# victorkich/ManyTor

Hardware: AMD Instinct MI355X
Metric: env-steps/sec (whole node), 1M parallel 4-DoF arms, random actions (higher is better)
Workload: dtype f32

## Files before the change

manytor_amd/csrc/engine.hip:

```cpp
#include <hip/hip_runtime.h>

#include <algorithm>
#include <cmath>
#include <cstdio>
#include <cstdlib>
#include <cstring>
#include <mutex>
#include <new>
#include <iterator>
#include <string>
#include <utility>
#include <vector>

#include "engine_internal.h"
#include "kernels.h"

using namespace mt;

namespace {
thread_local std::string g_last_error;
}

namespace mt {
int fail(mt_handle h, int code, const std::string& msg) {
  if (h)
    h->err = msg;
  else
    g_last_error = msg;
  return code;
}

int join_chains(mt_handle h) {
  if (!h->forked) return MT_OK;
  h->forked = false;
  for (int c = 1; c < mt_engine::kMaxChains; ++c) {
    if (!h->chain_streams[c] || !h->ev_join[c]) continue;
    MT_HIP(h, hipEventRecord(h->ev_join[c], h->chain_streams[c]));
    MT_HIP(h, hipStreamWaitEvent(h->stream, h->ev_join[c], 0));
  }
  return MT_OK;
}
}

namespace {

DhConst make_dh(const float* table, int dof) {
  DhConst t{};
  for (int j = 0; j < MT_MAX_DOF; ++j) {
    t.ca[j] = 1.f;
  }
  for (int j = 0; j < dof; ++j) {
    const double a = table[4 * j + 0], alpha = table[4 * j + 1], d = table[4 * j + 2], off = table[4 * j + 3];
    t.a[j] = (float)a;
    t.d[j] = (float)d;
    double sa = std::sin(alpha), ca = std::cos(alpha);
    if (std::fabs(sa) < 1e-7) sa = 0.0;
    if (std::fabs(ca) < 1e-7) ca = 0.0;
    t.sa[j] = (float)sa;
    t.ca[j] = (float)ca;
    t.off_deg[j] = (float)(off * 180.0 / M_PI);
  }
  t.fo = dof >= 2 ? dof - 2 : 0;
  t.fe = dof - 1;
  return t;
}

size_t align_up(size_t v, size_t a) { return (v + a - 1) / a * a; }

int ensure_staging(mt_handle h, size_t bytes) {
  if (h->staging_bytes >= bytes) return MT_OK;
  if (h->staging) {
    MT_HIP(h, hipStreamSynchronize(h->stream));
    MT_HIP(h, hipFree(h->staging));
    h->staging = nullptr;
    h->staging_bytes = 0;
  }
  if (hipMalloc(&h->staging, bytes) != hipSuccess) return fail(h, MT_ERR_ALLOC, "hipMalloc(staging) failed");
  h->staging_bytes = bytes;
  return MT_OK;
}

template <class Tbl>
bool table_matches(const DhConst& t, int dof) {
  if (dof != Tbl::D) return false;
  for (int j = 0; j < dof; ++j)
    if (t.a[j] != Tbl::a(j) || t.d[j] != Tbl::d(j) || t.sa[j] != Tbl::sa(j) || t.ca[j] != Tbl::ca(j) ||
        t.off_deg[j] != Tbl::off(j))
      return false;
  return true;
}

int match_static(const DhConst& t, int dof) {
  if (table_matches<Ref4Table>(t, dof)) return 1;
  if (table_matches<Dh7Table>(t, dof)) return 2;
  return 0;
}

struct BlockCap {
  int64_t from, below;
  int blocks;
};
struct DispatchPolicy {
  int64_t step_split4_max = 49152, step_split2_max = 65536;
  int64_t prefetch_other_max = 131072;
  int64_t fused_split4_max = 32768, fused_split2_max = 131072;
  int64_t reset_split_max = 65536;
  int64_t graph_max = 131072;
  int64_t chains_min = 163840, chains_max = 3145728;
  int64_t chain_split4_max = 16384, chain_split2_max = 49152, chain_prefetch_other_max = 131072;
  int64_t flat_from = 393216;
  BlockCap block_caps[3] = {{147456, 229376, 3}, {229376, 458752, 4}, {458752, 589824, 5}};
  int64_t multi_step_max = 262144;
  int multi_step_k = 5;
  bool fold_reset_into_chains = false;
  int max_recurrence_rotations = 12;
  int64_t ld_pad_above = 16384;
  int ld_pad_floats = 256;
};
static const DispatchPolicy kPolicy{};

static int step_blocks_per_cu(const mt_engine* h, int64_t n_launch) {
  if (h->blocks_per_cu_override >= 0) return h->blocks_per_cu_override;
  if (n_launch >= h->n) return 0;
  for (const BlockCap& c : kPolicy.block_caps)
    if (n_launch >= c.from && n_launch < c.below) return c.blocks;
  return 0;
}
static size_t lds_pad_for_blocks(int blocks_per_cu, size_t static_lds) {
  if (blocks_per_cu <= 0) return 0;
  const size_t per_block = (size_t)163840 / (size_t)blocks_per_cu - 1024;
  return per_block > static_lds ? std::min<size_t>(per_block, 65536) - static_lds : 0;
}

int64_t chain_span(const mt_engine* h, int chains) {
  const int64_t per = (h->n + chains - 1) / chains;
  return (per + 255) / 256 * 256;
}

static bool env_int(const char* name, long long* v) {
  const char* e = std::getenv(name);
  if (!e || !*e) return false;
  *v = std::atoll(e);
  return true;
}

static void choose_dispatch(mt_handle h) {
  const mt_config* cfg = &h->cfg;
  const DispatchPolicy& P = kPolicy;
  const int64_t n = cfg->n_envs;
  long long v = 0;
  h->overrides.clear();
  auto seen = [&](const char* name) { h->overrides += (h->overrides.empty() ? "" : ",") + std::string(name) + "=" + std::to_string(v); };

  h->trig = (cfg->flags & MT_FLAG_HW_TRIG) ? 2 : ((cfg->flags & MT_FLAG_DIRECT_TRIG) ? 1 : 0);
  if (cfg->flags & MT_FLAG_ABLATE_LOOP) h->trig = (cfg->flags & MT_FLAG_ABLATE_OBS) ? 4 : 3;
  else if (cfg->flags & MT_FLAG_ABLATE_OBS) h->trig = 5;
  const bool long_route = h->trig == 0 && (cfg->substeps - 1) / 2 > P.max_recurrence_rotations;
  if (long_route) h->trig = 1;
  h->lds_table = (cfg->flags & MT_FLAG_DH_IN_LDS) != 0 && !long_route;
  h->custom_frames = !(h->args.dh.fo == h->D - 2 && h->args.dh.fe == h->D - 1);
  h->static_kind = ((cfg->flags & (MT_FLAG_NO_SPECIALIZE | MT_FLAG_DH_IN_LDS)) || h->custom_frames) ? 0 : match_static(h->args.dh, h->D);

  int forced_lanes = 0, forced_prefetch = -1;
  if (env_int("MT_SPLIT", &v)) {
    forced_lanes = (v == 2 || v == 4) ? (int)v : 1;
    seen("MT_SPLIT");
  }
  if (env_int("MT_PREFETCH", &v)) {
    forced_prefetch = v != 0;
    seen("MT_PREFETCH");
  }
  h->reset_split = n <= P.reset_split_max;
  if (env_int("MT_RESET_SPLIT", &v)) {
    h->reset_split = v != 0;
    seen("MT_RESET_SPLIT");
  }
  h->graph_mode = -1;
  h->graph_max = P.graph_max;
  if (env_int("MT_GRAPH", &v)) {
    h->graph_mode = v != 0 ? 1 : 0;
    seen("MT_GRAPH");
  }
  h->flat_from = P.flat_from;
  if (env_int("MT_FLAT_FROM", &v)) {
    h->flat_from = std::max<long long>(0, v);
    seen("MT_FLAT_FROM");
  }
  h->blocks_per_cu_override = -1;
  if (env_int("MT_BLOCKS_PER_CU", &v)) {
    const int c = (int)std::max<long long>(0, std::min<long long>(8, v));
    h->blocks_per_cu_override = (c == 1 || c == 2) ? 3 : c;
    seen("MT_BLOCKS_PER_CU");
  }
  h->trig_steps = h->static_kind != 0;
  if (env_int("MT_TRIG_TABLE", &v)) {
    h->trig_steps = v != 0 && h->static_kind != 0;
    seen("MT_TRIG_TABLE");
  }

  h->chains = (n >= P.chains_min && n <= P.chains_max) ? 2 : 1;
  h->chains_forced = false;
  if (env_int("MT_CHAINS", &v)) {
    h->chains = (int)std::max<long long>(1, std::min<long long>(mt_engine::kMaxChains, v));
    h->chains_forced = true;
    seen("MT_CHAINS");
  }
  if (n < 2 * 256) h->chains = 1;
  h->lazy_chains = true;
  if (env_int("MT_LAZY_CHAINS", &v)) {
    h->lazy_chains = v != 0;
    seen("MT_LAZY_CHAINS");
  }

  h->multi_k = (n <= P.multi_step_max) ? P.multi_step_k : 1;
  if (env_int("MT_ROLLOUT_K", &v)) {
    h->multi_k = (int)std::max<long long>(1, std::min<long long>(64, v));
    seen("MT_ROLLOUT_K");
  }
  h->defer_reset = true;
  if (env_int("MT_DEFER_RESET", &v)) {
    h->defer_reset = v != 0;
    seen("MT_DEFER_RESET");
  }
  h->defer_reset_chained = P.fold_reset_into_chains;
  if (env_int("MT_DEFER_RESET_CHAINS", &v)) {
    h->defer_reset_chained = v != 0;
    seen("MT_DEFER_RESET_CHAINS");
  }
  h->gather_throttle = true;
  if (env_int("MT_GATHER_THROTTLE", &v)) {
    h->gather_throttle = v != 0;
    seen("MT_GATHER_THROTTLE");
  }
  h->snap_in_rollout = true;
  if (env_int("MT_ROLLOUT_SNAP", &v)) {
    h->snap_in_rollout = v != 0;
    seen("MT_ROLLOUT_SNAP");
  }
  h->rollout_early = true;
  if (env_int("MT_ROLLOUT_EARLY", &v)) {
    h->rollout_early = v != 0;
    seen("MT_ROLLOUT_EARLY");
  }

  h->tape_prefetch = false;
  if (env_int("MT_TAPE_PREFETCH", &v)) {
    h->tape_prefetch = v != 0;
    seen("MT_TAPE_PREFETCH");
  }
  h->tape_nt_loads = false;
  if (env_int("MT_TAPE_NT", &v)) {
    h->tape_nt_loads = v != 0;
    seen("MT_TAPE_NT");
  }

  h->ground_compact = true;
  if (env_int("MT_GROUND_COMPACT", &v)) {
    h->ground_compact = v != 0;
    seen("MT_GROUND_COMPACT");
  }

  if (h->custom_frames) h->lds_table = false;
  auto schedule_for = [&](int64_t envs, int64_t split4_max, int64_t split2_max, int64_t prefetch_other_max) {
    mt_engine::Schedule s;
    s.step_lanes = envs <= split4_max ? 4 : (envs <= split2_max ? 2 : 1);
    s.prefetch = h->static_kind == 1 || envs <= prefetch_other_max;
    s.rollout_lanes = envs <= P.fused_split4_max ? 4 : (envs <= P.fused_split2_max ? 2 : 1);
    if (forced_lanes) s.step_lanes = s.rollout_lanes = forced_lanes;
    if (forced_prefetch >= 0) s.prefetch = forced_prefetch != 0;
    if (h->custom_frames) s = mt_engine::Schedule{};
    return s;
  };
  h->sched[mt_engine::kBatch] = schedule_for(n, P.step_split4_max, P.step_split2_max, P.prefetch_other_max);
  h->sched[mt_engine::kChain] =
      h->chains > 1 ? schedule_for(chain_span(h, h->chains), P.chain_split4_max, P.chain_split2_max, P.chain_prefetch_other_max)
                    : h->sched[mt_engine::kBatch];
}

#define MT_DISPATCH_D(D_, FN, ...)   \
  switch (D_) {                      \
    case 2: FN<2>(__VA_ARGS__); break; \
    case 3: FN<3>(__VA_ARGS__); break; \
    case 4: FN<4>(__VA_ARGS__); break; \
    case 5: FN<5>(__VA_ARGS__); break; \
    case 6: FN<6>(__VA_ARGS__); break; \
    case 7: FN<7>(__VA_ARGS__); break; \
    case 8: FN<8>(__VA_ARGS__); break; \
    default: break;                  \
  }

struct StepVariant {
  int trig = 0;
  bool lds = false;
  int lanes = 1;
  int pf = 0;
  bool tt = false;
  bool flat = false;
  bool fresh = false;
  bool codes = false;
  bool gc = false;
};
constexpr unsigned variant_key(const StepVariant& v) {
  return (unsigned)v.trig | (unsigned)v.lds << 3 | (unsigned)v.lanes << 4 | (unsigned)(v.pf != 0) << 7 | (unsigned)v.tt << 8 |
         (unsigned)v.flat << 9 | (unsigned)v.fresh << 10 | (unsigned)v.codes << 11 | (unsigned)v.gc << 12;
}

#pragma clang diagnostic push
#pragma clang diagnostic ignored "-Wc++20-designator"
constexpr StepVariant kRuntimeVariants[] = {
    {.trig = 0}, {.trig = 1}, {.trig = 2}, {.trig = 3}, {.trig = 4}, {.trig = 5},
    {.lds = true},
    {.lanes = 2}, {.lanes = 4},
    {.pf = kPrefetch}, {.pf = kPrefetch, .flat = true},
    {.gc = true}, {.pf = kPrefetch, .gc = true}, {.pf = kPrefetch, .flat = true, .gc = true},
};
constexpr StepVariant kFramesVariants[] = {{.trig = 0}, {.trig = 1}};
constexpr StepVariant kStaticVariants[] = {
    {.trig = 0}, {.trig = 1}, {.trig = 2}, {.trig = 3}, {.trig = 4}, {.trig = 5},
    {.lanes = 2}, {.lanes = 4},
    {.lanes = 2, .tt = true}, {.lanes = 4, .tt = true},
    {.pf = kPrefetch}, {.pf = kPrefetch, .flat = true},
    {.pf = 0, .tt = true}, {.pf = kPrefetch, .tt = true}, {.pf = kPrefetch, .tt = true, .flat = true},
    {.pf = kPrefetch, .tt = true, .codes = true}, {.pf = kPrefetch, .tt = true, .flat = true, .codes = true},
    {.pf = 0, .tt = true, .fresh = true}, {.pf = kPrefetch, .tt = true, .fresh = true},
    {.pf = kPrefetch, .tt = true, .flat = true, .fresh = true},
    {.gc = true}, {.pf = kPrefetch, .gc = true}, {.pf = kPrefetch, .flat = true, .gc = true},
    {.pf = 0, .tt = true, .gc = true}, {.pf = kPrefetch, .tt = true, .gc = true}, {.pf = kPrefetch, .tt = true, .flat = true, .gc = true},
    {.pf = kPrefetch, .tt = true, .codes = true, .gc = true}, {.pf = kPrefetch, .tt = true, .flat = true, .codes = true, .gc = true},
};
#pragma clang diagnostic pop

enum class TableKind { kRuntime = 0, kRef4 = 1, kDh7 = 2, kFrames = 3 };
struct StepPlan {
  TableKind table = TableKind::kRuntime;
  int D = 0;
  bool sample = false;
  StepVariant v;
  int blocks_per_cu = 0;
  size_t lds_bytes = 0;
  dim3 grid;
  bool exists = true;
};

static bool ground_compacts(const mt_engine* h, bool whole_rows) {
  return h->ground_compact && whole_rows && h->trig == 0 && !h->lds_table && !h->custom_frames &&
         !(h->cfg.flags & MT_FLAG_DEBUG_ZMIN) && h->D <= 5;
}
template <int D>
static void ground_queue_bytes_d(size_t* out) { *out = sizeof(GroundQueue<RtTable<D>>); }
static size_t ground_queue_bytes(const mt_engine* h) {
  if (h->static_kind == 1) return sizeof(GroundQueue<Ref4Table>);
  if (h->static_kind == 2) return sizeof(GroundQueue<Dh7Table>);
  size_t bytes = 0;
  MT_DISPATCH_D(h->D, ground_queue_bytes_d, &bytes);
  return bytes;
}

StepPlan plan_step(const mt_engine* h, mt_engine::Scope scope, int64_t n, bool sample, bool codes, bool fresh = false) {
  const mt_engine::Schedule& s = h->sched[scope == mt_engine::kChain ? mt_engine::kChain : mt_engine::kBatch];
  const bool whole_rows = scope != mt_engine::kOneEnv;
  StepPlan p;
  p.table = h->custom_frames ? TableKind::kFrames : (TableKind)h->static_kind;
  p.D = h->D;
  p.sample = sample;
  p.grid = grid_for(n);
  StepVariant& v = p.v;
  if (fresh) {
    const size_t stage = (size_t)2 * h->K * kBlock * sizeof(float), fixed = kTrigEntries * sizeof(SinCos) + 512;
    p.exists = h->trig == 0 && h->trig_steps && s.step_lanes == 1 && !h->lds_table && !h->trace &&
               stage + fixed <= 65536;
    if (!p.exists) return p;
    p.sample = true;
    v.tt = v.fresh = true;
    v.pf = s.prefetch ? kPrefetch : 0;
    v.flat = v.pf && n >= h->flat_from;
    p.blocks_per_cu = v.pf ? step_blocks_per_cu(h, n) : 0;
    p.lds_bytes = std::max(stage, lds_pad_for_blocks(p.blocks_per_cu, fixed));
    return p;
  }
  if (p.table == TableKind::kFrames) {
    v.trig = h->trig == 1 ? 1 : 0;
    return p;
  }
  if (h->lds_table) {
    v.lds = true;
    return p;
  }
  if (h->trig != 0) {
    v.trig = h->trig;
    return p;
  }
  v.tt = sample && h->trig_steps && whole_rows;
  if (s.step_lanes > 1) {
    v.lanes = s.step_lanes;
    const int64_t per_block = kBlock / v.lanes;
    p.grid = dim3((unsigned)((n + per_block - 1) / per_block));
    return p;
  }
  v.pf = s.prefetch ? kPrefetch : 0;
  v.flat = v.pf && n >= h->flat_from;
  v.codes = v.pf && v.tt && codes;
  v.gc = ground_compacts(h, whole_rows);
  if (v.pf && v.tt) {
    p.blocks_per_cu = step_blocks_per_cu(h, n);
    p.lds_bytes = lds_pad_for_blocks(p.blocks_per_cu, kTrigEntries * sizeof(SinCos) + (v.gc ? ground_queue_bytes(h) : 0));
  }
  return p;
}

template <class Tbl, bool SAMPLE, const auto& ROWS, size_t I>
void launch_variant(const StepPlan& p, hipStream_t stream, const StepArgs& args) {
  constexpr StepVariant V = ROWS[I];
  if constexpr (V.lanes > 1)
    hipLaunchKernelGGL((step_split_kernel<Tbl, SAMPLE, V.lanes, V.tt>), p.grid, dim3(kBlock), p.lds_bytes, stream, args);
  else
    hipLaunchKernelGGL((step_kernel<Tbl, SAMPLE, V.trig, V.lds, V.pf, V.tt, V.flat, V.fresh, V.codes, V.gc>), p.grid, dim3(kBlock),
                       p.lds_bytes, stream, args);
}
template <class Tbl, const auto& ROWS, size_t I>
bool launch_row(const StepPlan& p, hipStream_t stream, const StepArgs& args) {
  if (variant_key(p.v) != variant_key(ROWS[I])) return false;
  if constexpr (ROWS[I].gc && Tbl::D >= 6)
    return false;
  else if (p.sample)
    launch_variant<Tbl, true, ROWS, I>(p, stream, args);
  else if constexpr (!ROWS[I].tt)
    launch_variant<Tbl, false, ROWS, I>(p, stream, args);
  else
    return false;
  return true;
}
template <class Tbl, const auto& ROWS, size_t... I>
bool launch_rows(const StepPlan& p, hipStream_t stream, const StepArgs& args, std::index_sequence<I...>) {
  return (launch_row<Tbl, ROWS, I>(p, stream, args) || ...);
}
template <class Tbl, const auto& ROWS>
bool launch_table(const StepPlan& p, hipStream_t stream, const StepArgs& args) {
  return launch_rows<Tbl, ROWS>(p, stream, args, std::make_index_sequence<std::size(ROWS)>{});
}
template <int D>
void launch_plan_d(const StepPlan& p, hipStream_t stream, const StepArgs& args, bool* launched) {
  *launched = p.table == TableKind::kFrames ? launch_table<RtTableF<D>, kFramesVariants>(p, stream, args)
                                            : launch_table<RtTable<D>, kRuntimeVariants>(p, stream, args);
}

void launch_plan(const StepPlan& p, hipStream_t stream, const StepArgs& args) {
  bool launched = false;
  if (p.v.gc && (int64_t)p.grid.x * kBlock > args.ld) {
    std::fprintf(stderr, "manytor: a ground-compacting step launch of %u blocks over rows of %lld\n", p.grid.x, (long long)args.ld);
    std::abort();
  }
  if (p.table == TableKind::kRef4)
    launched = launch_table<Ref4Table, kStaticVariants>(p, stream, args);
  else if (p.table == TableKind::kDh7)
    launched = launch_table<Dh7Table, kStaticVariants>(p, stream, args);
  else
    MT_DISPATCH_D(p.D, launch_plan_d, p, stream, args, &launched);
  if (!launched) {
    std::fprintf(stderr, "manytor: no step kernel for table %d, D %d, sample %d, variant key 0x%x\n", (int)p.table, p.D,
                 (int)p.sample, variant_key(p.v));
    std::abort();
  }
}

template <int D>
void launch_trace_d(mt_handle h, const StepArgs& args, float* trace, bool sample) {
  if (sample)
    hipLaunchKernelGGL((trace_kernel<D, true>), grid_for(args.n), dim3(kBlock), 0, h->stream, args, trace);
  else
    hipLaunchKernelGGL((trace_kernel<D, false>), grid_for(args.n), dim3(kBlock), 0, h->stream, args, trace);
}

void launch_step(mt_handle h, mt_engine::Scope scope, const StepArgs& args, float* trace, bool sample) {
  if (trace) MT_DISPATCH_D(h->D, launch_trace_d, h, args, trace, sample);
  const StepPlan p = plan_step(h, scope, args.n, sample, h->codes_valid);
  launch_plan(p, h->stream, args);
  h->codes_valid = p.v.codes;
}

void launch_step(mt_handle h, bool sample) { launch_step(h, mt_engine::kBatch, h->args, h->trace, sample); }

bool launch_step_fresh(mt_handle h, mt_engine::Scope scope, const StepArgs& args) {
  const StepPlan p = plan_step(h, scope, args.n, true, false, true);
  if (!p.exists) return false;
  launch_plan(p, h->stream, args);
  h->codes_valid = p.v.codes;
  return true;
}

StepArgs args_for_range(mt_handle h, const StepArgs& base, int64_t off, int64_t cnt);
int check_launch(mt_handle h, const char* what);
int ensure_chains(mt_handle h, int chains) {
  if (!h->ev_fork) MT_HIP(h, hipEventCreateWithFlags(&h->ev_fork, event_flags(false)));
  for (int c = 1; c < chains; ++c) {
    if (!h->chain_streams[c]) MT_HIP(h, hipStreamCreateWithFlags(&h->chain_streams[c], hipStreamNonBlocking));
    if (!h->ev_join[c]) MT_HIP(h, hipEventCreateWithFlags(&h->ev_join[c], event_flags(false)));
  }
  return MT_OK;
}

void launch_chain(mt_handle h, const StepArgs& a0, uint32_t major0, int T, int chains, int c, bool sample = true) {
  const int64_t span = chain_span(h, chains), off = (int64_t)c * span;
  if (off >= h->n) return;
  StepArgs as = args_for_range(h, a0, off, std::min(span, h->n - off));
  for (int s = 0; s < T; ++s) {
    as.major = major0 + (uint32_t)s;
    launch_step(h, mt_engine::kChain, as, nullptr, sample);
  }
}

bool launch_chain_fresh(mt_handle h, const StepArgs& a0, uint32_t major, int chains, int c) {
  const int64_t span = chain_span(h, chains), off = (int64_t)c * span;
  if (off >= h->n) return true;
  StepArgs as = args_for_range(h, a0, off, std::min(span, h->n - off));
  as.major = major;
  return launch_step_fresh(h, mt_engine::kChain, as);
}

hipStream_t chain_stream(mt_handle h, int c) { return c == 0 ? h->stream : h->chain_streams[c]; }

int fork_chains(mt_handle h, int chains) {
  if (h->forked) return MT_OK;
  int rc = ensure_chains(h, chains);
  if (rc) return rc;
  const int64_t span = chain_span(h, chains);
  MT_HIP(h, hipEventRecord(h->ev_fork, h->stream));
  for (int c = 1; c < chains; ++c)
    if ((int64_t)c * span < h->n) MT_HIP(h, hipStreamWaitEvent(h->chain_streams[c], h->ev_fork, 0));
  h->forked = true;
  return MT_OK;
}

int settle_chains(mt_handle h) { return (h->lazy_chains && h->stream == h->own_stream) ? MT_OK : join_chains(h); }

void shift_rows(StepArgs& a, int64_t off) {
  a.actions += off;
  a.goals += off;
  a.points += off;
  a.codes += off;
  a.alive += off;
  a.total_reward += off;
  a.obs += off;
  a.reward += off;
  a.done += off;
  a.ee += off;
  a.episodes += off;
  a.last_return += off;
  if (a.ring) a.ring += off;
  if (a.zmin) a.zmin += off;
  a.env_base += off;
}

StepArgs args_for_env(mt_handle h, int64_t env) {
  StepArgs a = h->args;
  shift_rows(a, env);
  a.done_bits = h->spare_bits;
  a.snap = nullptr;
  a.n = 1;
  return a;
}

StepArgs args_for_range(mt_handle h, const StepArgs& base, int64_t off, int64_t cnt) {
  StepArgs a = base;
  shift_rows(a, off);
  a.done_bits += off / 64;
  if (a.snap) a.snap += off;
  a.n = cnt;
  return a;
}

template <int D, bool RANDOM, bool ONLY_DONE>
void launch_reset_k(mt_handle h, const StepArgs& args) {
  const size_t lds = RANDOM ? (size_t)2 * args.K * kBlock * sizeof(float) : 0;
  if (lds > 65536)
    (void)hipFuncSetAttribute(reinterpret_cast<const void*>(&reset_kernel<D, RANDOM, ONLY_DONE>),
                              hipFuncAttributeMaxDynamicSharedMemorySize, (int)lds);
  hipLaunchKernelGGL((reset_kernel<D, RANDOM, ONLY_DONE>), grid_for(args.n), dim3(kBlock), lds, h->stream, args,
                     h->cfg.radius);
}
template <int D, bool ONLY_DONE>
void launch_reset_split(mt_handle h, const StepArgs& args) {
  constexpr int L = 4;
  const int64_t per_block = kBlock / L;
  const size_t lds = (size_t)2 * args.K * per_block * sizeof(float);
  hipLaunchKernelGGL((reset_split_kernel<D, ONLY_DONE, L>), dim3((unsigned)((args.n + per_block - 1) / per_block)),
                     dim3(kBlock), lds, h->stream, args, h->cfg.radius);
}
template <int D>
void launch_reset_d(mt_handle h, const StepArgs& args, int mode) {
  if (mode == 0) h->codes_valid = false;
  if (mode != 0 && h->reset_split && args.n == h->n)
    return mode == 1 ? launch_reset_split<D, false>(h, args) : launch_reset_split<D, true>(h, args);
  if (mode == 0)
    launch_reset_k<D, false, false>(h, args);
  else if (mode == 1)
    launch_reset_k<D, true, false>(h, args);
  else
    launch_reset_k<D, true, true>(h, args);
}

template <int D>
void launch_observe_d(mt_handle h) {
  hipLaunchKernelGGL((observe_kernel<D>), grid_for(h->n), dim3(kBlock), 0, h->stream, h->args);
}
template <int D>
void launch_check_done_d(mt_handle h) {
  hipLaunchKernelGGL((check_done_kernel<D>), grid_for(h->n), dim3(kBlock), 0, h->stream, h->args);
}
template <int D>
void launch_joints_d(mt_handle h, float* out) {
  hipLaunchKernelGGL((joints_kernel<D>), grid_for(h->n), dim3(kBlock), 0, h->stream, h->args, out);
}

template <class Tbl, int L, int RPF>
void launch_rollout_split_t(mt_handle h, const StepArgs& a, const RolloutArgs& r) {
  const int64_t per_block = kBlock / L;
  const size_t lds = (size_t)3 * h->K * per_block * sizeof(float) + (ActionTrigTable<Tbl>::value ? kTrigEntries * sizeof(SinCos) : 0);
  if (lds > 65536)
    (void)hipFuncSetAttribute(reinterpret_cast<const void*>(&rollout_split_kernel<Tbl, L, RPF>),
                              hipFuncAttributeMaxDynamicSharedMemorySize, (int)lds);
  hipLaunchKernelGGL((rollout_split_kernel<Tbl, L, RPF>), dim3((unsigned)((a.n + per_block - 1) / per_block)), dim3(kBlock), lds,
                     h->stream, a, r);
}

template <class Tbl, int RPF>
void launch_rollout_t(mt_handle h, const StepArgs& a, int lanes, const RolloutArgs& r) {
  if (lanes == 4) return launch_rollout_split_t<Tbl, 4, RPF>(h, a, r);
  if (lanes == 2) return launch_rollout_split_t<Tbl, 2, RPF>(h, a, r);
  const size_t lds = (size_t)3 * h->K * kBlock * sizeof(float) + (ActionTrigTable<Tbl>::value ? kTrigEntries * sizeof(SinCos) : 0);
  if (lds > 65536)
    (void)hipFuncSetAttribute(reinterpret_cast<const void*>(&rollout_kernel<Tbl, RPF>),
                              hipFuncAttributeMaxDynamicSharedMemorySize, (int)lds);
  hipLaunchKernelGGL((rollout_kernel<Tbl, RPF>), grid_for(a.n), dim3(kBlock), lds, h->stream, a, r);
}

template <int D>
void launch_rollout_d(mt_handle h, const StepArgs& a, int lanes, const RolloutArgs& r) {
  launch_rollout_t<RtTable<D>, 0>(h, a, lanes, r);
}
void launch_rollout(mt_handle h, const StepArgs& a, int lanes, const RolloutArgs& r, bool early = false) {
  h->codes_valid = false;
  if (h->static_kind == 1) return early ? launch_rollout_t<Ref4Table, kPrefetch>(h, a, lanes, r) : launch_rollout_t<Ref4Table, 0>(h, a, lanes, r);
  if (h->static_kind == 2) return early ? launch_rollout_t<Dh7Table, kPrefetch>(h, a, lanes, r) : launch_rollout_t<Dh7Table, 0>(h, a, lanes, r);
  MT_DISPATCH_D(h->D, launch_rollout_d, h, a, lanes, r);
}

template <class Tbl, bool PREFETCH>
void launch_tape_t(mt_handle h, const StepArgs& a, const TapeArgs& r) {
  const size_t lds = (size_t)3 * h->K * kBlock * sizeof(float);
  if (lds > 65536)
    (void)hipFuncSetAttribute(reinterpret_cast<const void*>(&rollout_tape_kernel<Tbl, PREFETCH>),
                              hipFuncAttributeMaxDynamicSharedMemorySize, (int)lds);
  hipLaunchKernelGGL((rollout_tape_kernel<Tbl, PREFETCH>), grid_for(a.n), dim3(kBlock), lds, h->stream, a, r);
}
template <int D>
void launch_tape_d(mt_handle h, const StepArgs& a, const TapeArgs& r) {
  launch_tape_t<RtTable<D>, false>(h, a, r);
}
bool tape_prefetches(const mt_engine* h) { return h->tape_prefetch && h->static_kind != 0; }
void launch_tape(mt_handle h, const StepArgs& a, const TapeArgs& r) {
  const bool pf = tape_prefetches(h);
  if (h->static_kind == 1) return pf ? launch_tape_t<Ref4Table, true>(h, a, r) : launch_tape_t<Ref4Table, false>(h, a, r);
  if (h->static_kind == 2) return pf ? launch_tape_t<Dh7Table, true>(h, a, r) : launch_tape_t<Dh7Table, false>(h, a, r);
  MT_DISPATCH_D(h->D, launch_tape_d, h, a, r);
}

template <class Tbl>
struct TableTag {
  using type = Tbl;
};
template <class F>
void with_table(const mt_engine* h, F&& f) {
  if (h->static_kind == 1) return f(TableTag<Ref4Table>{});
  if (h->static_kind == 2) return f(TableTag<Dh7Table>{});
  switch (h->D) {
    case 2: return f(TableTag<RtTable<2>>{});
    case 3: return f(TableTag<RtTable<3>>{});
    case 4: return f(TableTag<RtTable<4>>{});
    case 5: return f(TableTag<RtTable<5>>{});
    case 6: return f(TableTag<RtTable<6>>{});
    case 7: return f(TableTag<RtTable<7>>{});
    case 8: return f(TableTag<RtTable<8>>{});
    default: return;
  }
}

template <class Tbl>
void launch_tape_select_t(mt_handle h, const StepArgs& a, const TapeArgs& r) {
  const size_t lds = (size_t)3 * h->K * kBlock * sizeof(float);
  if (lds > 65536)
    (void)hipFuncSetAttribute(reinterpret_cast<const void*>(&rollout_tape_kernel<Tbl, false, true>),
                              hipFuncAttributeMaxDynamicSharedMemorySize, (int)lds);
  hipLaunchKernelGGL((rollout_tape_kernel<Tbl, false, true>), grid_for(a.n), dim3(kBlock), lds, h->stream, a, r);
}
void launch_tape_select(mt_handle h, const StepArgs& a, const TapeArgs& r) {
  with_table(h, [&](auto tag) { launch_tape_select_t<typename decltype(tag)::type>(h, a, r); });
}

template <class Tbl, int W>
void launch_policy_t(mt_handle h, const StepArgs& a, const PolicyArgs& r) {
  const size_t lds = (size_t)3 * h->K * kBlock * sizeof(float);
  if (lds > 65536)
    (void)hipFuncSetAttribute(reinterpret_cast<const void*>(&rollout_policy_kernel<Tbl, W>),
                              hipFuncAttributeMaxDynamicSharedMemorySize, (int)lds);
  hipLaunchKernelGGL((rollout_policy_kernel<Tbl, W>), grid_for(a.n), dim3(kBlock), lds, h->stream, a, r);
}
void launch_policy(mt_handle h, const StepArgs& a, const PolicyArgs& r, int width) {
  with_table(h, [&](auto tag) {
    using Tbl = typename decltype(tag)::type;
    if (width <= 32) return launch_policy_t<Tbl, 32>(h, a, r);
    launch_policy_t<Tbl, 64>(h, a, r);
  });
}


template <class Tbl>
void launch_shoot_t(mt_handle h, const StepArgs& a, const ShootArgs& r) {
  const size_t lds = ((size_t)3 * h->K + 2 * kShootWaves) * kShootEnvs * sizeof(float);
  hipLaunchKernelGGL((shoot_kernel<Tbl>), dim3((unsigned)((a.n + kShootEnvs - 1) / kShootEnvs)), dim3(kBlock), lds, h->stream, a, r);
}
void launch_shoot(mt_handle h, const StepArgs& a, const ShootArgs& r) {
  with_table(h, [&](auto tag) { launch_shoot_t<typename decltype(tag)::type>(h, a, r); });
}

template <class Tbl>
void launch_cem_t(mt_handle h, const StepArgs& a, const CemArgs& r) {
  const size_t lds = ((size_t)3 * h->K + (size_t)r.C + 2 * kShootWaves + 1) * kShootEnvs * sizeof(float);
  hipLaunchKernelGGL((cem_kernel<Tbl>), dim3((unsigned)((a.n + kShootEnvs - 1) / kShootEnvs)), dim3(kBlock), lds, h->stream, a, r);
}
void launch_cem(mt_handle h, const StepArgs& a, const CemArgs& r) {
  with_table(h, [&](auto tag) { launch_cem_t<typename decltype(tag)::type>(h, a, r); });
}

template <class Tbl>
void launch_mppi_t(mt_handle h, const StepArgs& a, const MppiArgs& r) {
  const size_t lds = (((size_t)3 * h->K + (size_t)r.C) * kShootEnvs + kMppiTable) * sizeof(float);
  hipLaunchKernelGGL((mppi_kernel<Tbl>), dim3((unsigned)((a.n + kShootEnvs - 1) / kShootEnvs)), dim3(kBlock), lds, h->stream, a, r);
}
void launch_mppi(mt_handle h, const StepArgs& a, const MppiArgs& r) {
  with_table(h, [&](auto tag) { launch_mppi_t<typename decltype(tag)::type>(h, a, r); });
}

template <int D>
void launch_sample_plans_d(mt_handle h, const CemArgs& r, float* plans, int64_t ld, int64_t cand_stride) {
  hipLaunchKernelGGL((sample_plans_kernel<D>), dim3(grid_for(h->n).x, (unsigned)r.T, (unsigned)r.C), dim3(kBlock), 0, h->stream, r, plans,
                     ld, cand_stride, h->args.n, h->args.env_base);
}

bool fusable(mt_handle h) { return h->trig == 0 && !h->lds_table && !h->trace && !h->custom_frames; }
const char* unfusable_reason(const mt_engine* h) {
  return h->custom_frames                        ? "custom obs_frame / ee_frame"
         : h->trace                              ? "MT_FLAG_TRACE"
         : h->lds_table                          ? "MT_FLAG_DH_IN_LDS"
         : h->trig == 2                          ? "MT_FLAG_HW_TRIG"
         : (h->cfg.flags & MT_FLAG_DIRECT_TRIG) ? "MT_FLAG_DIRECT_TRIG"
         : h->trig == 1                          ? "substeps beyond the recurrence's reach (per-pose trigonometry)"
                                                 : "a profiling flag (MT_FLAG_ABLATE_*)";
}
int fail_unfusable(mt_handle h, const char* who) {
  return fail(h, MT_ERR_UNSUPPORTED, std::string(who) + ": not available on a handle with " + unfusable_reason(h));
}

bool rollout_is_multi_step(mt_handle h) { return h->multi_k > 1 && fusable(h); }
bool chained_rollout_absorbs_reset(mt_handle h) {
  const bool graph = h->graph_mode > 0 || (h->graph_mode < 0 && h->n <= h->graph_max);
  return h->defer_reset_chained && !rollout_is_multi_step(h) && h->chains > 1 && h->lazy_chains && !h->trace && !graph && fusable(h);
}


int check_launch(mt_handle h, const char* what) {
  hipError_t e = hipGetLastError();
  if (e != hipSuccess) return fail(h, MT_ERR_HIP, std::string(what) + " launch: " + hipGetErrorString(e));
  return MT_OK;
}

struct FieldInfo {
  void* ptr;
  int rows;
  int dtype;
  size_t esize;
};

int field_info(mt_handle h, int field, FieldInfo* fi) {
  const StepArgs& a = h->args;
  switch (field) {
    case MT_F_ACTIONS: *fi = {a.actions, h->D, MT_F32, 4}; return MT_OK;
    case MT_F_GOALS: *fi = {a.goals, h->D, MT_F32, 4}; return MT_OK;
    case MT_F_POINTS: *fi = {a.points, 3 * h->K, MT_F32, 4}; return MT_OK;
    case MT_F_ALIVE: *fi = {a.alive, 1, MT_U32, 4}; return MT_OK;
    case MT_F_OBS: *fi = {a.obs, 3 * h->K, MT_F32, 4}; return MT_OK;
    case MT_F_REWARD: *fi = {a.reward, 1, MT_I32, 4}; return MT_OK;
    case MT_F_DONE: *fi = {a.done, 1, MT_U8, 1}; return MT_OK;
    case MT_F_DONE_BITS: *fi = {a.done_bits, 1, MT_U64, 8}; return MT_OK;
    case MT_F_EE: *fi = {a.ee, 3, MT_F32, 4}; return MT_OK;
// ... 262 lines not shown
  };
#define MT_HIP_C(call)                                                                       \
  do {                                                                                       \
    hipError_t e__ = (call);                                                                 \
    if (e__ != hipSuccess) return bail(MT_ERR_HIP, std::string(#call) + ": " + hipGetErrorString(e__)); \
  } while (0)

  DeviceGuard guard(cfg->device);
  if (guard.error() != hipSuccess) return bail(MT_ERR_HIP, std::string("hipSetDevice: ") + hipGetErrorString(guard.error()));
  MT_HIP_C(hipStreamCreateWithFlags(&h->own_stream, hipStreamNonBlocking));
  h->stream = h->own_stream;
  MT_HIP_C(hipEventCreateWithFlags(&h->ev0, event_flags(true)));
  MT_HIP_C(hipEventCreateWithFlags(&h->ev1, event_flags(true)));

  const size_t ld = (size_t)h->ld, D = (size_t)h->D, K = (size_t)h->K;
  size_t off = 0;
  auto take = [&](size_t bytes) {
    size_t o = off;
    off = align_up(off + bytes, 1024);
    return o;
  };
  const size_t o_act = take(D * ld * 4), o_goal = take(D * ld * 4), o_pts = take(3 * K * ld * 4),
               o_obs = take(3 * K * ld * 4), o_alive = take(ld * 4), o_tot = take(ld * 4), o_rew = take(ld * 4),
               o_done = take(ld), o_bits = take(ld / 64 * 8), o_ee = take(3 * ld * 4), o_epi = take(ld * 4),
               o_last = take(ld * 4), o_ring = take((size_t)cfg->return_ring * ld * 4), o_misc = take(256),
               o_trace = take((cfg->flags & MT_FLAG_TRACE) ? (size_t)cfg->substeps * 3 * ld * 4 : 0),
               o_zmin = take((cfg->flags & MT_FLAG_DEBUG_ZMIN) ? ld * 4 : 0), o_trig = take(kTrigEntries * sizeof(SinCos)),
               o_codes = take(2 * K * ld * 4);
  h->arena_bytes = off;
  if (hipMalloc(&h->arena, h->arena_bytes) != hipSuccess) {
    (void)hipGetLastError();
    return bail(MT_ERR_ALLOC, "hipMalloc of the state arena failed (" + std::to_string(h->arena_bytes) + " bytes)");
  }
  MT_HIP_C(hipMemsetAsync(h->arena, 0, h->arena_bytes, h->stream));
  char* base = (char*)h->arena;
  StepArgs& a = h->args;
  a.actions = (float*)(base + o_act);
  a.goals = (float*)(base + o_goal);
  a.points = (float*)(base + o_pts);
  a.codes = (uint32_t*)(base + o_codes);
  a.obs = (float*)(base + o_obs);
  a.alive = (uint32_t*)(base + o_alive);
  a.total_reward = (float*)(base + o_tot);
  a.reward = (int32_t*)(base + o_rew);
  a.done = (uint8_t*)(base + o_done);
  a.done_bits = (unsigned long long*)(base + o_bits);
  a.ee = (float*)(base + o_ee);
  a.episodes = (uint32_t*)(base + o_epi);
  a.last_return = (float*)(base + o_last);
  a.ring = cfg->return_ring ? (float*)(base + o_ring) : nullptr;
  a.ring_slots = (uint32_t)cfg->return_ring;
  a.episode0 = 0;
  a.bad_actions = (uint32_t*)(base + o_misc);
  h->spare_bits = (unsigned long long*)(base + o_misc + 64);
  h->trace = (cfg->flags & MT_FLAG_TRACE) ? (float*)(base + o_trace) : nullptr;
  a.zmin = (cfg->flags & MT_FLAG_DEBUG_ZMIN) ? (float*)(base + o_zmin) : nullptr;
  a.snap = nullptr;
  a.trig_table = (const float*)(base + o_trig);
  hipLaunchKernelGGL(fill_trig_table_kernel, dim3(1), dim3(kBlock), 0, h->stream, (float*)(base + o_trig));
  MT_HIP_C(hipGetLastError());
  a.n = h->n;
  a.ld = h->ld;
  a.env_base = cfg->env_id_base;
  a.K = h->K;
  a.S = cfg->substeps;
  a.tol = cfg->pickup_tol;
  a.radius = cfg->radius;
  a.inv_sm1 = 1.0f / (float)(cfg->substeps - 1);
  a.flags = cfg->flags & ~kFlagWholeGoals;
  a.dh = make_dh(cfg->dh_table, h->D);
  a.dh.fo = (cfg->obs_frame + h->D) % h->D;
  a.dh.fe = (cfg->ee_frame + h->D) % h->D;
  choose_dispatch(h);
#undef MT_HIP_C
  *out = h;
  return MT_OK;
}

int mt_destroy(mt_handle h) {
  if (!h) return MT_OK;
  DeviceGuard guard(h->cfg.device);
  (void)hipStreamSynchronize(h->stream);
  mt_gather_release(h);
  mt_comm_release(h);
  for (auto& g : h->graphs)
    for (hipGraphExec_t x : g.exec)
      if (x) (void)hipGraphExecDestroy(x);
  for (int c = 1; c < mt_engine::kMaxChains; ++c) {
    if (h->chain_streams[c]) {
      (void)hipStreamSynchronize(h->chain_streams[c]);
      (void)hipStreamDestroy(h->chain_streams[c]);
    }
    if (h->ev_join[c]) (void)hipEventDestroy(h->ev_join[c]);
    if (h->ev1c[c]) (void)hipEventDestroy(h->ev1c[c]);
  }
  if (h->ev_fork) (void)hipEventDestroy(h->ev_fork);
  if (h->graph_step0) (void)hipFree(h->graph_step0);
  if (h->staging) (void)hipFree(h->staging);
  if (h->pinned) (void)hipHostFree(h->pinned);
  if (h->arena) (void)hipFree(h->arena);
  if (h->ev0) (void)hipEventDestroy(h->ev0);
  if (h->ev1) (void)hipEventDestroy(h->ev1);
  for (hipEvent_t e : h->lap_events) (void)hipEventDestroy(e);
  if (h->own_stream) (void)hipStreamDestroy(h->own_stream);
  delete h;
  return MT_OK;
}

static StepPlan batch_plan(const mt_engine* h) { return plan_step(h, mt_engine::kBatch, h->n, true, false); }
static StepPlan chain_plan(const mt_engine* h) { return plan_step(h, mt_engine::kChain, chain_span(h, h->chains), true, false); }
static std::string table_name(const mt_engine* h) {
  const char* tbl = h->static_kind == 1 ? "Ref4Table" : (h->static_kind == 2 ? "Dh7Table" : nullptr);
  return tbl ? tbl : (h->custom_frames ? "RtTableF<" : "RtTable<") + std::to_string(h->D) + ">";
}
static int multi_step_lanes(const mt_engine* h) {
  return h->sched[(h->chains > 1 && h->chains_forced) ? mt_engine::kChain : mt_engine::kBatch].rollout_lanes;
}

const char* mt_step_kernel_name(mt_handle h) {
  if (!h) return "";
  const std::string table = table_name(h);
  const StepVariant v = batch_plan(h).v;
  if (v.lanes > 1)
    h->kernel_name = "step_split_kernel<" + table + ", L=" + std::to_string(v.lanes) + (v.tt ? ", tt=1>" : ">");
  else
    h->kernel_name = "step_kernel<" + table + ", trig=" + std::to_string(h->trig) + ", lds=" + (v.lds ? "true" : "false") +
                     ", pf=" + std::to_string(v.pf) + (v.tt ? ", tt=1" : "") + (v.flat ? ", flat=1>" : ">");
  const bool multi_one_chain = h->multi_k > 1 && fusable(h) && !h->chains_forced;
  if (h->chains > 1 && !multi_one_chain) {
    const StepPlan c = chain_plan(h);
    h->kernel_name += " [mt_rollout: " + std::to_string(h->chains) + " chains of " + std::to_string(chain_span(h, h->chains)) +
                      " envs, " + (c.v.lanes > 1 ? "L=" + std::to_string(c.v.lanes)
                                                 : "pf=" + std::to_string(c.v.pf) + (c.v.flat ? ", flat=1" : "")) +
                      (c.blocks_per_cu > 0 ? ", " + std::to_string(c.blocks_per_cu) + " blocks/CU" : std::string()) + "]";
  }
  if (h->multi_k > 1 && fusable(h)) {
    const int sp = multi_step_lanes(h);
    h->kernel_name += " [mt_rollout: " + std::to_string(h->multi_k) + " steps per launch, " +
                      (sp > 1 ? "rollout_split_kernel L=" + std::to_string(sp) : std::string("rollout_kernel")) + "]";
  }
  return h->kernel_name.c_str();
}

const char* mt_describe_dispatch(mt_handle h) {
  if (!h) return "";
  const DispatchPolicy& P = kPolicy;
  auto num = [](long long v) { return std::to_string(v); };
  auto b = [](bool v) { return std::string(v ? "true" : "false"); };
  const int64_t span = chain_span(h, h->chains);
  const std::string table = table_name(h);
  const StepPlan sb = batch_plan(h), sc = chain_plan(h);
  const bool multi = h->multi_k > 1 && fusable(h);
  const bool graph = h->graph_mode > 0 || (h->graph_mode < 0 && h->n <= h->graph_max);
  std::string caps = "[";
  for (const BlockCap& c : P.block_caps) caps += std::string(caps.size() > 1 ? "," : "") + "[" + num(c.from) + "," + num(c.below) + "," + num(c.blocks) + "]";
  caps += "]";
  std::string& d = h->describe;
  d = "{\"n_envs\":" + num(h->n) + ",\"ld\":" + num(h->ld) + ",\"dof\":" + num(h->D) + ",\"targets\":" + num(h->K) +
      ",\"table\":\"" + table + "\",\"trig\":" + num(h->trig) + ",\"lds_table\":" + b(h->lds_table) + ",\"custom_frames\":" + b(h->custom_frames) +
      ",\"step\":{\"lanes_per_env\":" + num(sb.v.lanes) + ",\"prefetch\":" + b(sb.v.pf != 0) +
      ",\"trig_table\":" + b(sb.v.tt) + ",\"flat\":" + b(sb.v.flat) + "}" +
      ",\"chains\":{\"count\":" + num(h->chains) + ",\"span\":" + num(h->chains > 1 ? span : h->n) + ",\"lazy\":" + b(h->lazy_chains) +
      ",\"lanes_per_env\":" + num(sc.v.lanes) + ",\"prefetch\":" + b(sc.v.pf != 0) + ",\"flat\":" + b(sc.v.flat) +
      ",\"blocks_per_cu\":" + num(h->chains > 1 ? sc.blocks_per_cu : 0) + "}" +
      ",\"rollout\":{\"form\":\"" + (multi ? "multi_step" : (h->chains > 1 ? "chained_steps" : (graph ? "graph_replay" : "launch_per_step"))) +
      "\",\"steps_per_launch\":" + num(multi ? h->multi_k : 1) + ",\"graph\":" + b(!multi && graph) +
      ",\"lanes_per_env\":" + num(multi ? multi_step_lanes(h) : (h->chains > 1 ? sc : sb).v.lanes) +
      ",\"chains\":" + num(multi && !h->chains_forced ? 1 : h->chains) +
      ",\"absorbs_reset\":" + b(h->defer_reset && (multi || chained_rollout_absorbs_reset(h))) + ",\"writes_snapshot\":" + b(h->snap_in_rollout && (multi || (h->chains > 1 && !graph && !h->trace))) + "}" +
      ",\"fused\":{\"usable\":" + b(fusable(h)) + ",\"lanes_per_env\":" + num(h->sched[mt_engine::kBatch].rollout_lanes) + "}" +
      ",\"tape\":{\"usable\":" + b(fusable(h)) + ",\"lanes_per_env\":1,\"chains\":1,\"prefetch\":" + b(tape_prefetches(h)) +
      ",\"nt_loads\":" + b(h->tape_nt_loads) + "}" +
      ",\"shoot\":{\"usable\":" + b(fusable(h)) + ",\"envs_per_block\":" + num(kShootEnvs) + ",\"waves_per_block\":" + num(kShootWaves) + "}" +
      ",\"cem\":{\"usable\":" + b(fusable(h)) + ",\"envs_per_block\":" + num(kShootEnvs) + ",\"waves_per_block\":" + num(kShootWaves) +
      ",\"max_candidates\":64}" +
      ",\"mppi\":{\"usable\":" + b(fusable(h)) + ",\"envs_per_block\":" + num(kShootEnvs) + ",\"waves_per_block\":" + num(kShootWaves) +
      ",\"max_candidates\":64,\"max_steps\":" + num(kMppiMaxSteps) + "}" +
      ",\"policy_rollout\":{\"usable\":" + b(fusable(h)) + ",\"lanes_per_env\":1,\"hidden_extents\":[32,64]}" +
      ",\"reset\":{\"lanes_per_env\":" + num(h->reset_split ? 4 : 1) + "}" +
      ",\"ground_compact\":{\"enabled\":" + b(h->ground_compact) + ",\"step\":" + b(sb.v.gc) + ",\"chains\":" + b(sc.v.gc) + "}" +
      ",\"overrides\":\"" + h->overrides + "\"" +
      ",\"policy\":{\"step_split4_max\":" + num(P.step_split4_max) + ",\"step_split2_max\":" + num(P.step_split2_max) +
      ",\"prefetch_other_max\":" + num(P.prefetch_other_max) + ",\"fused_split4_max\":" + num(P.fused_split4_max) +
      ",\"fused_split2_max\":" + num(P.fused_split2_max) + ",\"reset_split_max\":" + num(P.reset_split_max) +
      ",\"graph_max\":" + num(P.graph_max) + ",\"chains_min\":" + num(P.chains_min) + ",\"chains_max\":" + num(P.chains_max) +
      ",\"chain_split4_max\":" + num(P.chain_split4_max) + ",\"chain_split2_max\":" + num(P.chain_split2_max) +
      ",\"chain_prefetch_other_max\":" + num(P.chain_prefetch_other_max) + ",\"flat_from\":" + num(P.flat_from) +
      ",\"block_caps\":" + caps + ",\"multi_step_max\":" + num(P.multi_step_max) + ",\"multi_step_k\":" + num(P.multi_step_k) +
      ",\"max_recurrence_rotations\":" + num(P.max_recurrence_rotations) + ",\"ld_pad_above\":" + num(P.ld_pad_above) +
      ",\"ld_pad_floats\":" + num(P.ld_pad_floats) + "}" +
      ",\"arena_bytes\":" + num((long long)h->arena_bytes) + "}";
  return d.c_str();
}

int mt_set_stream(mt_handle h, void* hip_stream) {
  MT_REQUIRE(nullptr, h != nullptr, "handle is NULL");
  MT_ENTER(h);
  MT_HIP(h, hipStreamSynchronize(h->stream));
  h->stream = (hipStream_t)hip_stream;
  return MT_OK;
}

int mt_use_own_stream(mt_handle h) {
  MT_REQUIRE(nullptr, h != nullptr, "handle is NULL");
  MT_ENTER(h);
  MT_HIP(h, hipStreamSynchronize(h->stream));
  h->stream = h->own_stream;
  return MT_OK;
}

int mt_sync(mt_handle h) {
  MT_REQUIRE(nullptr, h != nullptr, "handle is NULL");
  MT_ENTER(h);
  MT_HIP(h, hipStreamSynchronize(h->stream));
  if (h->gather_pending) {
    MT_HIP(h, hipStreamSynchronize(h->side_stream));
    MT_HIP(h, hipEventElapsedTime(&h->last_gather_ms, h->ev_g0, h->ev_g1));
    h->gather_pending = false;
    h->snap_free_known[0] = h->snap_free_known[1] = true;
  }
  return MT_OK;
}

int mt_reset(mt_handle h, const float* points, int layout, int is_device) {
  MT_REQUIRE(nullptr, h != nullptr, "handle is NULL");
  MT_REQUIRE(h, points != nullptr, "points is NULL (use mt_reset_random for device-drawn targets)");
  MT_REQUIRE(h, layout == MT_ENV_MAJOR || layout == MT_SOA, "bad layout");
  if (!is_device && layout == MT_ENV_MAJOR) {
    const int64_t bad = first_unusable(points, h->n * 3 * h->K, kMaxFiniteBits);
    if (bad >= 0) return fail(h, MT_ERR_INVALID_ARG, "mt_reset: points element " + std::to_string(bad) + " is NaN or infinite");
  }
  if (!is_device && layout == MT_SOA)
    for (int r = 0; r < 3 * h->K; ++r) {
      const int64_t bad = first_unusable(points + (int64_t)r * h->ld, h->n, kMaxFiniteBits);
      if (bad >= 0)
        return fail(h, MT_ERR_INVALID_ARG, "mt_reset: points row " + std::to_string(r) + " element " + std::to_string(bad) + " is NaN or infinite");
    }
  MT_ENTER(h);
  const int rows = 3 * h->K;
  if (layout == MT_SOA) {
    const size_t bytes = (size_t)rows * h->ld * 4;
    MT_HIP(h, hipMemcpyAsync(h->args.points, points, bytes, is_device ? hipMemcpyDeviceToDevice : hipMemcpyHostToDevice,
                             h->stream));
  } else {
    const size_t bytes = (size_t)rows * h->n * 4;
    const float* src = points;
    if (!is_device) {
      int rc = ensure_staging(h, bytes);
      if (rc) return rc;
      MT_HIP(h, hipMemcpyAsync(h->staging, points, bytes, hipMemcpyHostToDevice, h->stream));
      src = (const float*)h->staging;
    }
    hipLaunchKernelGGL((env_major_to_soa<float>), grid_for(h->n), dim3(kBlock), 0, h->stream, src, rows, h->n,
                       h->args.points, h->ld);
    int rc = check_launch(h, "env_major_to_soa");
    if (rc) return rc;
  }
  {
    int rcg = order_behind_inplace_gather(h, h->stream);
    if (rcg) return rcg;
  }
  h->args.major = 0;
  h->args.episode0 = 0;
  if (!h->goals_exposed) h->args.flags |= kFlagWholeGoals;
  MT_DISPATCH_D(h->D, launch_reset_d, h, h->args, 0);
  int rc = check_launch(h, "reset_kernel");
  if (rc) return rc;
  if (!is_device) MT_HIP(h, hipStreamSynchronize(h->stream));
  h->is_reset = true;
  return MT_OK;
}

static int launch_reset_random(mt_handle h, uint64_t seed, uint32_t episode, int mode) {
  const bool per_chain = mode == 1 && h->chains > 1 && h->lazy_chains && h->forked;
  if (!per_chain) {
    int rc = join_chains(h);
    if (rc) return rc;
  }
  h->args.seed_lo = (uint32_t)seed;
  h->args.seed_hi = (uint32_t)(seed >> 32);
  h->args.major = episode;
  if (mode == 1) {
    h->args.episode0 = episode;
    if (!h->goals_exposed) h->args.flags |= kFlagWholeGoals;
  }
  if (per_chain) {
    int rc = fork_chains(h, h->chains);
    if (rc) return rc;
    const int64_t span = chain_span(h, h->chains);
    hipStream_t root = h->stream;
    for (int c = 0; c < h->chains && rc == MT_OK; ++c) {
      const int64_t off = (int64_t)c * span;
      if (off >= h->n) continue;
      const StepArgs ar = args_for_range(h, h->args, off, std::min(span, h->n - off));
      h->stream = c == 0 ? root : h->chain_streams[c];
      rc = order_behind_inplace_gather(h, h->stream);
      if (rc == MT_OK) MT_DISPATCH_D(h->D, launch_reset_d, h, ar, 1);
    }
    h->stream = root;
    if (rc == MT_OK) rc = check_launch(h, "reset_kernel (per chain)");
    if (rc) return rc;
    h->codes_valid = !h->points_exposed;
    h->is_reset = true;
    return settle_chains(h);
  }
  int rc = order_behind_inplace_gather(h, h->stream);
  if (rc) return rc;
  MT_DISPATCH_D(h->D, launch_reset_d, h, h->args, mode);
  rc = check_launch(h, "reset_kernel");
  if (rc) return rc;
  if (mode == 1) h->codes_valid = !h->points_exposed;
  h->is_reset = true;
  return MT_OK;
}

}

namespace mt {
int flush_pending_reset(mt_handle h) {
  if (!h->reset_pending) return MT_OK;
  h->reset_pending = false;
  return launch_reset_random(h, h->pend_seed, h->pend_episode, 1);
}
}

extern "C" {

static int reset_random_impl(mt_handle h, uint64_t seed, uint32_t episode, int mode) {
  MT_REQUIRE(nullptr, h != nullptr, "handle is NULL");
  MT_ON_DEVICE(h, h->cfg.device);
  h->snap_valid = false;
  int rc = flush_pending_reset(h);
  if (rc) return rc;
  if (mode == 1 && h->defer_reset && h->stream == h->own_stream &&
      ((rollout_is_multi_step(h) && !h->forked) || chained_rollout_absorbs_reset(h))) {
    h->args.seed_lo = (uint32_t)seed;
    h->args.seed_hi = (uint32_t)(seed >> 32);
    h->args.major = episode;
    h->args.episode0 = episode;
    if (!h->goals_exposed) h->args.flags |= kFlagWholeGoals;
    h->reset_pending = true;
    h->pend_seed = seed;
    h->pend_episode = episode;
    h->is_reset = true;
    return MT_OK;
  }
  return launch_reset_random(h, seed, episode, mode);
}

int mt_reset_random(mt_handle h, uint64_t seed, uint32_t episode) { return reset_random_impl(h, seed, episode, 1); }

int mt_reset_done(mt_handle h, uint64_t seed) {
  MT_REQUIRE(nullptr, h != nullptr, "handle is NULL");
  if (!h->is_reset) return fail(h, MT_ERR_STATE, "mt_reset_done before the first reset");
  return reset_random_impl(h, seed, 0, 2);
}

int mt_set_actions(mt_handle h, const void* actions, int dtype, int layout, int is_device) {
  MT_REQUIRE(nullptr, h != nullptr, "handle is NULL");
  MT_REQUIRE(h, actions != nullptr, "actions is NULL");
  MT_REQUIRE(h, layout == MT_ENV_MAJOR || layout == MT_SOA, "bad layout");
  MT_REQUIRE(h, dtype == MT_F32 || dtype == MT_F64 || dtype == MT_I32 || dtype == MT_I64, "bad action dtype");
  const size_t es = (dtype == MT_F32 || dtype == MT_I32) ? 4 : 8;
  const int chains = is_device ? usable_chains(h, true) : 1;
  if (chains > 1) {
    MT_ON_DEVICE(h, h->cfg.device);
    const int D = h->D;
    const int64_t ld = h->ld;
    hipError_t copy_err = hipSuccess;
    int rc = per_chain(h, chains, "set_actions (per chain)", [&](int, int64_t off, int64_t cnt) {
      const dim3 g = grid_for(cnt), b(kBlock);
      float* dst = h->args.actions + off;
      if (layout == MT_SOA && dtype == MT_F32) {
        hipError_t e = hipMemcpy2DAsync(dst, (size_t)ld * 4, (const float*)actions + off, (size_t)ld * 4, (size_t)cnt * 4, (size_t)D,
                                        hipMemcpyDeviceToDevice, h->stream);
        if (e != hipSuccess) copy_err = e;
      } else if (layout == MT_ENV_MAJOR) {
        const char* src = (const char*)actions + (size_t)off * D * es;
        switch (dtype) {
          case MT_F32: hipLaunchKernelGGL((env_major_to_soa<float>), g, b, 0, h->stream, (const float*)src, D, cnt, dst, ld); break;
          case MT_F64: hipLaunchKernelGGL((env_major_to_soa<double>), g, b, 0, h->stream, (const double*)src, D, cnt, dst, ld); break;
          case MT_I32: hipLaunchKernelGGL((env_major_to_soa<int32_t>), g, b, 0, h->stream, (const int32_t*)src, D, cnt, dst, ld); break;
          default: hipLaunchKernelGGL((env_major_to_soa<int64_t>), g, b, 0, h->stream, (const int64_t*)src, D, cnt, dst, ld); break;
        }
      } else {
        const char* src = (const char*)actions + (size_t)off * es;
        switch (dtype) {
          case MT_F64: hipLaunchKernelGGL((soa_to_soa_f32<double>), g, b, 0, h->stream, (const double*)src, D, cnt, ld, dst); break;
          case MT_I32: hipLaunchKernelGGL((soa_to_soa_f32<int32_t>), g, b, 0, h->stream, (const int32_t*)src, D, cnt, ld, dst); break;
          default: hipLaunchKernelGGL((soa_to_soa_f32<int64_t>), g, b, 0, h->stream, (const int64_t*)src, D, cnt, ld, dst); break;
        }
      }
    });
    if (rc) return rc;
    if (copy_err != hipSuccess) return fail(h, MT_ERR_HIP, std::string("hipMemcpy2DAsync (actions): ") + hipGetErrorString(copy_err));
    return MT_OK;
  }
  MT_ENTER(h);
  const int64_t cols = (layout == MT_SOA) ? h->ld : h->n;
  const size_t bytes = (size_t)h->D * cols * es;
  const void* src = actions;
  if (layout == MT_SOA && dtype == MT_F32) {
    MT_HIP(h, hipMemcpyAsync(h->args.actions, actions, bytes,
                             is_device ? hipMemcpyDeviceToDevice : hipMemcpyHostToDevice, h->stream));
    if (!is_device) MT_HIP(h, hipStreamSynchronize(h->stream));
    return MT_OK;
  }
  if (!is_device) {
    int rc = ensure_staging(h, bytes);
    if (rc) return rc;
    MT_HIP(h, hipMemcpyAsync(h->staging, actions, bytes, hipMemcpyHostToDevice, h->stream));
    src = h->staging;
  }
  const dim3 g = grid_for(h->n), b(kBlock);
  if (layout == MT_ENV_MAJOR) {
    switch (dtype) {
      case MT_F32: hipLaunchKernelGGL((env_major_to_soa<float>), g, b, 0, h->stream, (const float*)src, h->D, h->n, h->args.actions, h->ld); break;
      case MT_F64: hipLaunchKernelGGL((env_major_to_soa<double>), g, b, 0, h->stream, (const double*)src, h->D, h->n, h->args.actions, h->ld); break;
      case MT_I32: hipLaunchKernelGGL((env_major_to_soa<int32_t>), g, b, 0, h->stream, (const int32_t*)src, h->D, h->n, h->args.actions, h->ld); break;
      default: hipLaunchKernelGGL((env_major_to_soa<int64_t>), g, b, 0, h->stream, (const int64_t*)src, h->D, h->n, h->args.actions, h->ld); break;
    }
  } else {
    switch (dtype) {
      case MT_F64: hipLaunchKernelGGL((soa_to_soa_f32<double>), g, b, 0, h->stream, (const double*)src, h->D, h->n, h->ld, h->args.actions); break;
      case MT_I32: hipLaunchKernelGGL((soa_to_soa_f32<int32_t>), g, b, 0, h->stream, (const int32_t*)src, h->D, h->n, h->ld, h->args.actions); break;
      default: hipLaunchKernelGGL((soa_to_soa_f32<int64_t>), g, b, 0, h->stream, (const int64_t*)src, h->D, h->n, h->ld, h->args.actions); break;
    }
  }
  int rc = check_launch(h, "set_actions");
  if (rc) return rc;
  if (!is_device) MT_HIP(h, hipStreamSynchronize(h->stream));
  return MT_OK;
}

int mt_sample_actions(mt_handle h, uint64_t seed, uint32_t step_idx) {
  MT_REQUIRE(nullptr, h != nullptr, "handle is NULL");
  const int chains = usable_chains(h, true);
  if (chains > 1) {
    MT_ON_DEVICE(h, h->cfg.device);
    return per_chain(h, chains, "sample_actions_kernel (per chain)", [&](int, int64_t off, int64_t cnt) {
      hipLaunchKernelGGL(sample_actions_kernel, grid_for(cnt), dim3(kBlock), 0, h->stream, h->args.actions + off, cnt, h->ld, h->D,
                         h->args.env_base + off, seed, step_idx);
    });
  }
  MT_ENTER(h);
  hipLaunchKernelGGL(sample_actions_kernel, grid_for(h->n), dim3(kBlock), 0, h->stream, h->args.actions, h->n, h->ld,
                     h->D, h->args.env_base, seed, step_idx);
  return check_launch(h, "sample_actions_kernel");
}

int mt_step(mt_handle h) {
  MT_REQUIRE(nullptr, h != nullptr, "handle is NULL");
  if (!h->is_reset) return fail(h, MT_ERR_STATE, "mt_step before mt_reset / mt_reset_random");
  const int chains = usable_chains(h, true);
  if (chains > 1) {
    MT_ON_DEVICE(h, h->cfg.device);
    h->snap_valid = false;
    {
      int rcf = flush_pending_reset(h);
      if (rcf) return rcf;
    }
    const StepArgs a = h->args;
    int rc = per_chain(h, chains, "step_kernel (per chain)", [&](int c, int64_t, int64_t) { launch_chain(h, a, a.major, 1, chains, c, false); });
    h->args.flags &= ~kFlagWholeGoals;
    return rc;
  }
  MT_ENTER(h);
  launch_step(h, false);
  h->args.flags &= ~kFlagWholeGoals;
  return check_launch(h, "step_kernel");
}

int mt_step_host(mt_handle h, const void* actions, int dtype, float* obs, int32_t* reward, uint8_t* done) {
  MT_REQUIRE(nullptr, h != nullptr, "handle is NULL");
  MT_REQUIRE(h, actions && obs && reward && done, "NULL argument");
  MT_REQUIRE(h, dtype == MT_F32 || dtype == MT_F64 || dtype == MT_I32 || dtype == MT_I64, "bad action dtype");
  if (!h->is_reset) return fail(h, MT_ERR_STATE, "mt_step_host before mt_reset / mt_reset_random");
  MT_ENTER(h);
  const size_t n = (size_t)h->n, es = (dtype == MT_F32 || dtype == MT_I32) ? 4 : 8;
  const size_t in_b = n * h->D * es, obs_b = n * 3 * h->K * 4, rew_b = n * 4, done_b = n;
  const size_t out_b = obs_b + rew_b + done_b, total = align_up(in_b, 256) + out_b;
  if (h->pinned_bytes < total) {
    if (h->pinned) {
      MT_HIP(h, hipStreamSynchronize(h->stream));
      (void)hipHostFree(h->pinned);
      h->pinned = nullptr;
      h->pinned_bytes = 0;
    }
    if (hipHostMalloc(&h->pinned, total, hipHostMallocDefault) != hipSuccess) {
      (void)hipGetLastError();
      return fail(h, MT_ERR_ALLOC, "hipHostMalloc failed");
    }
    h->pinned_bytes = total;
  }
  int rc = ensure_staging(h, total);
  if (rc) return rc;
  char* hp = (char*)h->pinned;
  char* dp = (char*)h->staging;
  char* hp_out = hp + align_up(in_b, 256);
  char* dp_out = dp + align_up(in_b, 256);
  std::memcpy(hp, actions, in_b);
  MT_HIP(h, hipMemcpyAsync(dp, hp, in_b, hipMemcpyHostToDevice, h->stream));
  const dim3 g = grid_for(h->n), b(kBlock);
  switch (dtype) {
    case MT_F32: hipLaunchKernelGGL((env_major_to_soa<float>), g, b, 0, h->stream, (const float*)dp, h->D, h->n, h->args.actions, h->ld); break;
    case MT_F64: hipLaunchKernelGGL((env_major_to_soa<double>), g, b, 0, h->stream, (const double*)dp, h->D, h->n, h->args.actions, h->ld); break;
    case MT_I32: hipLaunchKernelGGL((env_major_to_soa<int32_t>), g, b, 0, h->stream, (const int32_t*)dp, h->D, h->n, h->args.actions, h->ld); break;
    default: hipLaunchKernelGGL((env_major_to_soa<int64_t>), g, b, 0, h->stream, (const int64_t*)dp, h->D, h->n, h->args.actions, h->ld); break;
  }
  launch_step(h, false);
  h->args.flags &= ~kFlagWholeGoals;
  hipLaunchKernelGGL((soa_to_env_major<float>), g, b, 0, h->stream, h->args.obs, h->ld, 3 * h->K, h->n, (float*)dp_out);
  rc = check_launch(h, "mt_step_host");
  if (rc) return rc;
  MT_HIP(h, hipMemcpyAsync(dp_out + obs_b, h->args.reward, rew_b, hipMemcpyDeviceToDevice, h->stream));
  MT_HIP(h, hipMemcpyAsync(dp_out + obs_b + rew_b, h->args.done, done_b, hipMemcpyDeviceToDevice, h->stream));
  MT_HIP(h, hipMemcpyAsync(hp_out, dp_out, out_b, hipMemcpyDeviceToHost, h->stream));
  MT_HIP(h, hipStreamSynchronize(h->stream));
  std::memcpy(obs, hp_out, obs_b);
  std::memcpy(reward, hp_out + obs_b, rew_b);
  std::memcpy(done, hp_out + obs_b + rew_b, done_b);
  return MT_OK;
}

int mt_step_random(mt_handle h, uint64_t seed, uint32_t step_idx) {
  MT_REQUIRE(nullptr, h != nullptr, "handle is NULL");
  if (!h->is_reset) return fail(h, MT_ERR_STATE, "mt_step_random before mt_reset / mt_reset_random");
  MT_ENTER(h);
  h->args.seed_lo = (uint32_t)seed;
  h->args.seed_hi = (uint32_t)(seed >> 32);
  h->args.major = step_idx;
  launch_step(h, true);
  return check_launch(h, "step_kernel");
}

static int rebuild_done_word(mt_handle h, int64_t env) {
  hipLaunchKernelGGL(done_bits_word_kernel, dim3(1), dim3(64), 0, h->stream, h->args.done, h->n, env >> 6,
                     h->args.done_bits);
  return check_launch(h, "done_bits_word_kernel");
}

int mt_env_step(mt_handle h, int64_t env, const float* action, float* obs, int32_t* reward, uint8_t* done) {
  MT_REQUIRE(nullptr, h != nullptr, "handle is NULL");
  MT_REQUIRE(h, action && obs && reward && done, "NULL argument");
  MT_REQUIRE(h, env >= 0 && env < h->n, "env index out of range");
  if (!h->is_reset) return fail(h, MT_ERR_STATE, "mt_env_step before mt_reset / mt_reset_random");
  MT_ENTER(h);
  const StepArgs a = args_for_env(h, env);
  const size_t pitch = (size_t)h->ld * 4;
  MT_HIP(h, hipMemcpy2DAsync(a.actions, pitch, action, 4, 4, (size_t)h->D, hipMemcpyHostToDevice, h->stream));
  launch_step(h, mt_engine::kOneEnv, a, h->trace ? h->trace + env : nullptr, false);
  h->args.flags &= ~kFlagWholeGoals;
  int rc = check_launch(h, "step_kernel (one env)");
  if (rc) return rc;
  rc = rebuild_done_word(h, env);
  if (rc) return rc;
  MT_HIP(h, hipMemcpy2DAsync(obs, 4, a.obs, pitch, 4, (size_t)(3 * h->K), hipMemcpyDeviceToHost, h->stream));
  MT_HIP(h, hipMemcpyAsync(reward, a.reward, 4, hipMemcpyDeviceToHost, h->stream));
  MT_HIP(h, hipMemcpyAsync(done, a.done, 1, hipMemcpyDeviceToHost, h->stream));
  MT_HIP(h, hipStreamSynchronize(h->stream));
  return MT_OK;
}

int mt_env_reset(mt_handle h, int64_t env, const float* points, uint64_t seed, uint32_t episode) {
  MT_REQUIRE(nullptr, h != nullptr, "handle is NULL");
  MT_REQUIRE(h, env >= 0 && env < h->n, "env index out of range");
  if (!h->is_reset) return fail(h, MT_ERR_STATE, "mt_env_reset before the first reset of the batch");
  if (points && first_unusable(points, 3 * (int64_t)h->K, kMaxFiniteBits) >= 0)
    return fail(h, MT_ERR_INVALID_ARG, "mt_env_reset: a target coordinate is NaN or infinite");
  MT_ENTER(h);
  StepArgs a = args_for_env(h, env);
  if (points)
    MT_HIP(h, hipMemcpy2DAsync(a.points, (size_t)h->ld * 4, points, 4, 4, (size_t)(3 * h->K), hipMemcpyHostToDevice,
                               h->stream));
  a.seed_lo = (uint32_t)seed;
  a.seed_hi = (uint32_t)(seed >> 32);
  a.major = episode;
  {
    int rcg = order_behind_inplace_gather(h, h->stream);
    if (rcg) return rcg;
  }
  MT_DISPATCH_D(h->D, launch_reset_d, h, a, points ? 0 : 1);
  int rc = check_launch(h, "reset_kernel (one env)");
  if (rc) return rc;
  rc = rebuild_done_word(h, env);
  if (rc) return rc;
  MT_HIP(h, hipStreamSynchronize(h->stream));
  return MT_OK;
}

int mt_bad_action_count(mt_handle h, uint64_t* count) {
  MT_REQUIRE(nullptr, h != nullptr, "handle is NULL");
  MT_REQUIRE(h, count != nullptr, "count is NULL");
  MT_ENTER(h);
  uint32_t c = 0;
  MT_HIP(h, hipMemcpyAsync(&c, h->args.bad_actions, 4, hipMemcpyDeviceToHost, h->stream));
  MT_HIP(h, hipStreamSynchronize(h->stream));
  *count = c;
  return MT_OK;
}

static bool rollout_uses_graph(mt_handle h, int n_steps) {
  if (h->graph_mode == 0 || h->trace || n_steps < 4) return false;
  if (h->graph_mode < 0 && h->n > h->graph_max) return false;

  hipStreamCaptureStatus st = hipStreamCaptureStatusNone;
  if (hipStreamIsCapturing(h->stream, &st) != hipSuccess || st != hipStreamCaptureStatusNone) {
    (void)hipGetLastError();
    return false;
  }
  return true;
}

static int rollout_graph(mt_handle h, int T, uint64_t seed, int chains, const mt_engine::RolloutGraph** out) {
  if (!h->graph_step0) MT_HIP(h, hipMalloc(&h->graph_step0, sizeof(uint32_t) * mt_engine::kMaxChains));
  StepArgs a = h->args;
  a.seed_lo = (uint32_t)seed;
  a.seed_hi = (uint32_t)(seed >> 32);
  a.major = 0;
  a.episode0 = 0;
  a.major_base = h->graph_step0;
  for (auto& g : h->graphs)
    if (g.T == T && g.chains == chains && std::memcmp(&g.args, &a, sizeof a) == 0) {
      *out = &g;
      return MT_OK;
    }
  mt_engine::RolloutGraph rg{};
  rg.T = T;
  rg.chains = chains;
  rg.args = a;
  hipStream_t launch_stream = h->stream;
  auto drop = [&]() {
    for (int c = 0; c < chains; ++c)
      if (rg.exec[c]) (void)hipGraphExecDestroy(rg.exec[c]);
  };
  for (int c = 0; c < chains; ++c) {
    if (c > 0 && (int64_t)c * chain_span(h, chains) >= h->n) break;
    hipGraph_t graph = nullptr;
    MT_HIP(h, hipStreamBeginCapture(h->own_stream, hipStreamCaptureModeThreadLocal));
    h->stream = h->own_stream;
    if (chains > 1) {
      StepArgs ac = a;
      ac.major_base = h->graph_step0 + c;
      launch_chain(h, ac, 0u, T, chains, c);
    } else {
      for (int s = 0; s < T; ++s) {
        StepArgs as = a;
        as.major = (uint32_t)s;
        launch_step(h, mt_engine::kBatch, as, nullptr, true);
      }
    }
    h->stream = launch_stream;
    hipError_t e = hipStreamEndCapture(h->own_stream, &graph);
    if (e != hipSuccess || !graph) {
      (void)hipGetLastError();
      drop();
      return fail(h, MT_ERR_HIP, std::string("mt_rollout: stream capture failed: ") + hipGetErrorString(e));
    }
    e = hipGraphInstantiate(&rg.exec[c], graph, nullptr, nullptr, 0);
    (void)hipGraphDestroy(graph);
    if (e != hipSuccess) {
      rg.exec[c] = nullptr;
      drop();
      return fail(h, MT_ERR_HIP, std::string("hipGraphInstantiate: ") + hipGetErrorString(e));
    }
  }
  if (h->graphs.size() >= 8) {
    int rcj = join_chains(h);
    if (rcj) return rcj;
    MT_HIP(h, hipStreamSynchronize(h->stream));
    for (int c = 1; c < mt_engine::kMaxChains; ++c)
      if (h->chain_streams[c]) MT_HIP(h, hipStreamSynchronize(h->chain_streams[c]));
    for (hipGraphExec_t x : h->graphs.front().exec)
      if (x) (void)hipGraphExecDestroy(x);
    h->graphs.erase(h->graphs.begin());
  }
  h->graphs.push_back(rg);
  *out = &h->graphs.back();
  return MT_OK;
}

int mt_rollout(mt_handle h, int n_steps, uint64_t seed, uint32_t step_idx0) {
  MT_REQUIRE(nullptr, h != nullptr, "handle is NULL");
  MT_REQUIRE(h, n_steps >= 0, "n_steps must be >= 0");
  if (n_steps > 0 && !h->is_reset) return fail(h, MT_ERR_STATE, "mt_rollout before mt_reset / mt_reset_random");
  if (n_steps == 0) return MT_OK;
  MT_ON_DEVICE(h, h->cfg.device);
  int chains = (n_steps >= 2 || h->reset_pending) ? usable_chains(h) : 1;
  h->snap_valid = false;
  const bool multi = (n_steps >= 2 || h->reset_pending) && rollout_is_multi_step(h);
  const bool chained_fresh = h->reset_pending && !multi && chains > 1 && chained_rollout_absorbs_reset(h) && !rollout_uses_graph(h, n_steps);
  if (n_steps < 2 && !multi && !chained_fresh) chains = 1;
  if (h->reset_pending && !multi && !chained_fresh) {
    int rc = flush_pending_reset(h);
    if (rc) return rc;
  }
  if (multi) {
    if (!h->chains_forced) chains = 1;
    StepArgs a = h->args;
    a.seed_lo = (uint32_t)seed;
    a.seed_hi = (uint32_t)(seed >> 32);
    const bool fresh = h->reset_pending;
    h->reset_pending = false;
    bool snap = h->snap_in_rollout && h->snap != nullptr && snapshot_trusted(h);
    const int snap_p = h->snap_next;
    if (snap && !h->snap_free_known[snap_p]) {
      if (hipEventQuery(h->ev_gdone[snap_p]) == hipSuccess) {
        h->snap_free_known[snap_p] = true;
      } else {
        (void)hipGetLastError();
        snap = false;
      }
    }
    auto args_of = [&](int s0) {
      RolloutArgs r{std::min(h->multi_k, n_steps - s0), step_idx0 + (uint32_t)s0, 0u, h->cfg.radius, 0u, 0u, 0u, 0u, nullptr};
      if (fresh && s0 == 0) {
        r.reset_first = 1u;
        r.reset_episode = h->pend_episode;
        r.reset_seed_lo = (uint32_t)h->pend_seed;
        r.reset_seed_hi = (uint32_t)(h->pend_seed >> 32);
      }
      if (snap && s0 + h->multi_k >= n_steps) r.snap = h->snap_row(snap_p);
      return r;
    };
    int rc = MT_OK;
    if (fresh) {
      rc = order_behind_inplace_gather(h, h->stream);
      if (rc) return rc;
    }
    if (chains > 1) {
      rc = fork_chains(h, chains);
      if (rc) return rc;
      const int64_t span = chain_span(h, chains);
      hipStream_t root = h->stream;
      for (int s0 = 0; s0 < n_steps; s0 += h->multi_k) {
        for (int c = 0; c < chains; ++c) {
          const int64_t off = (int64_t)c * span;
          if (off >= h->n) continue;
          h->stream = c == 0 ? root : h->chain_streams[c];
          RolloutArgs r = args_of(s0);
          if (r.snap) r.snap += off;
          if (fresh && s0 == 0 && c > 0 && rc == MT_OK) rc = order_behind_inplace_gather(h, h->stream);
          if (rc == MT_OK) launch_rollout(h, args_for_range(h, a, off, std::min(span, h->n - off)), h->sched[mt_engine::kChain].rollout_lanes, r, h->rollout_early);
        }
      }
      h->stream = root;
      if (rc == MT_OK) rc = check_launch(h, "rollout_kernel (mt_rollout, per chain)");
      if (rc) return rc;
      rc = settle_chains(h);
    } else {
      rc = join_chains(h);
      if (rc) return rc;
      for (int s0 = 0; s0 < n_steps; s0 += h->multi_k) launch_rollout(h, a, h->sched[mt_engine::kBatch].rollout_lanes, args_of(s0), h->rollout_early);
      rc = check_launch(h, "rollout_kernel (mt_rollout)");
    }
    if (rc) return rc;
    h->snap_valid = snap;
    h->args.seed_lo = (uint32_t)seed;
    h->args.seed_hi = (uint32_t)(seed >> 32);
    h->args.major = step_idx0 + (uint32_t)(n_steps - 1);
    return MT_OK;
  }
  bool graph = rollout_uses_graph(h, n_steps);
  if (graph && h->graph_mode < 0) {
    bool cached = false, seen = false;
    for (auto& g : h->graphs) cached |= g.T == n_steps;
    for (int t : h->graph_seen) seen |= t == n_steps;
    if (!cached && !seen) {
      if (h->graph_seen.size() >= 32) h->graph_seen.erase(h->graph_seen.begin());
      h->graph_seen.push_back(n_steps);
      graph = false;
    }
  }
  if (chains == 1) {
    int rc = join_chains(h);
    if (rc) return rc;
  }
  if (graph) {
    const mt_engine::RolloutGraph* rg = nullptr;
    h->codes_valid = false;
    int rc = rollout_graph(h, n_steps, seed, chains, &rg);
    if (rc) return rc;
    if (chains > 1) {
      rc = fork_chains(h, chains);
      if (rc) return rc;
      const int64_t span = chain_span(h, chains);
      for (int c = 0; c < chains; ++c) {
        if ((int64_t)c * span >= h->n) continue;
        MT_HIP(h, hipMemsetD32Async((hipDeviceptr_t)(h->graph_step0 + c), (int)step_idx0, 1, chain_stream(h, c)));
        MT_HIP(h, hipGraphLaunch(rg->exec[c], chain_stream(h, c)));
      }
      rc = settle_chains(h);
      if (rc) return rc;
    } else {
      MT_HIP(h, hipMemsetD32Async((hipDeviceptr_t)h->graph_step0, (int)step_idx0, 1, h->stream));
      MT_HIP(h, hipGraphLaunch(rg->exec[0], h->stream));
    }
  } else if (chains > 1) {
    StepArgs a = h->args;
    a.seed_lo = (uint32_t)seed;
    a.seed_hi = (uint32_t)(seed >> 32);
    int rc = fork_chains(h, chains);
    if (rc) return rc;
    hipStream_t root = h->stream;
    const int64_t span = chain_span(h, chains);
    h->reset_pending = false;
    StepArgs a_last = a;
    {
      const int sp = h->snap_next;
      bool snap = h->snap_in_rollout && h->snap != nullptr && !h->trace && snapshot_trusted(h);
      if (snap && !h->snap_free_known[sp]) {
        if (hipEventQuery(h->ev_gdone[sp]) == hipSuccess) {
          h->snap_free_known[sp] = true;
        } else {
          (void)hipGetLastError();
          snap = false;
        }
      }
      if (snap) a_last.snap = h->snap_row(sp);
    }
    bool fresh_by_rollout_kernel = false;
    for (int st = 0; st < n_steps; ++st)
      for (int c = 0; c < chains; ++c) {
        h->stream = c == 0 ? root : h->chain_streams[c];
        const int64_t off = (int64_t)c * span;
        if (chained_fresh && st == 0 && off < h->n) {
          if (rc == MT_OK) rc = order_behind_inplace_gather(h, h->stream);
          if (rc != MT_OK) continue;
          StepArgs af = (n_steps == 1) ? a_last : a;
          af.reset_seed_lo = (uint32_t)h->pend_seed;
          af.reset_seed_hi = (uint32_t)(h->pend_seed >> 32);
          af.reset_episode = h->pend_episode;
          af.radius = h->cfg.radius;
          if (launch_chain_fresh(h, af, step_idx0, chains, c)) continue;
          fresh_by_rollout_kernel = true;
          const RolloutArgs r{1, step_idx0, 0u, h->cfg.radius, 1u, h->pend_episode, (uint32_t)h->pend_seed, (uint32_t)(h->pend_seed >> 32), nullptr};
          launch_rollout(h, args_for_range(h, a, off, std::min(span, h->n - off)), 1, r, h->rollout_early);
          continue;
        }
        if (rc == MT_OK) launch_chain(h, st == n_steps - 1 ? a_last : a, step_idx0 + (uint32_t)st, 1, chains, c);
      }
    h->stream = root;
    if (rc == MT_OK) rc = check_launch(h, "step_kernel (chained)");
    if (rc) return rc;
    rc = settle_chains(h);
    if (rc) return rc;
    h->snap_valid = a_last.snap != nullptr && !(fresh_by_rollout_kernel && n_steps == 1);
  } else {
    for (int s = 0; s < n_steps; ++s) {
      int rc = mt_step_random(h, seed, step_idx0 + (uint32_t)s);
      if (rc) return rc;
    }
    return MT_OK;
  }
  h->args.seed_lo = (uint32_t)seed;
  h->args.seed_hi = (uint32_t)(seed >> 32);
  h->args.major = step_idx0 + (uint32_t)(n_steps - 1);
  return MT_OK;
}

int mt_rollout_fused(mt_handle h, int n_steps, uint64_t seed, uint32_t step_idx0, int auto_reset) {
  MT_REQUIRE(nullptr, h != nullptr, "handle is NULL");
  MT_REQUIRE(h, n_steps >= 0, "n_steps must be >= 0");
  if (!h->is_reset) return fail(h, MT_ERR_STATE, "mt_rollout_fused before mt_reset / mt_reset_random");
  if (n_steps == 0) return MT_OK;
  if (!fusable(h)) {
    for (int s = 0; s < n_steps; ++s) {
      int rc = mt_step_random(h, seed, step_idx0 + (uint32_t)s);
      if (rc) return rc;
      if (auto_reset) {
        rc = mt_reset_done(h, seed);
        if (rc) return rc;
      }
    }
    return MT_OK;
  }
  MT_ENTER(h);
  h->args.seed_lo = (uint32_t)seed;
  h->args.seed_hi = (uint32_t)(seed >> 32);
  if (auto_reset) {
    int rcg = order_behind_inplace_gather(h, h->stream);
    if (rcg) return rcg;
  }
  RolloutArgs r{n_steps, step_idx0, auto_reset ? 1u : 0u, h->cfg.radius, 0u, 0u, 0u, 0u, nullptr};
  launch_rollout(h, h->args, h->sched[mt_engine::kBatch].rollout_lanes, r);
  return check_launch(h, "rollout_kernel");
}

int mt_rollout_tape(mt_handle h, const mt_tape* tape) {
  MT_REQUIRE(nullptr, h != nullptr, "handle is NULL");
  MT_REQUIRE(h, tape != nullptr, "tape is NULL");
  MT_REQUIRE(h, tape->struct_size == (int32_t)sizeof(mt_tape), "mt_tape.struct_size does not match this library");
  MT_REQUIRE(h, tape->reserved == 0, "mt_tape.reserved must be 0");
  MT_REQUIRE(h, (tape->flags & ~(MT_TAPE_AUTO_RESET | MT_TAPE_DRY_RUN)) == 0, "unknown MT_TAPE_* flag");
  const bool auto_reset = (tape->flags & MT_TAPE_AUTO_RESET) != 0, dry = (tape->flags & MT_TAPE_DRY_RUN) != 0;
  MT_REQUIRE(h, !(auto_reset && dry), "MT_TAPE_DRY_RUN | MT_TAPE_AUTO_RESET: the re-arm writes the return ring");
  MT_REQUIRE(h, tape->n_steps >= 0, "n_steps must be >= 0");
  if (!fusable(h)) return fail_unfusable(h, "mt_rollout_tape");
  if (!h->is_reset) return fail(h, MT_ERR_STATE, "mt_rollout_tape before mt_reset / mt_reset_random");
  if (tape->n_steps == 0) return MT_OK;
  MT_REQUIRE(h, tape->actions != nullptr, "mt_tape.actions is NULL");
  MT_REQUIRE(h, tape->ld >= h->n, "mt_tape.ld is smaller than n_envs");
  MT_REQUIRE(h, !(tape->reward_log || tape->done_log) || tape->log_ld >= h->n, "mt_tape.log_ld is smaller than n_envs");
  MT_ENTER(h);
  TapeArgs r = tape_args(tape, tape->actions, tape->ld, tape->n_steps);
  r.dry_run = dry ? 1u : 0u;
  r.nt_loads = h->tape_nt_loads ? 1u : 0u;
  return commit_tape(h, r, tape->seed, auto_reset, false);
}

struct PolicyScreen {
  int widest = 0;
  bool noisy = false;
};
static int rollout_policy_screen(mt_handle h, const struct mt_policy* p, const std::string& nm, const char* who, PolicyScreen* out) {
  MT_REQUIRE(h, (p->flags & ~(MT_POLICY_AUTO_RESET | MT_POLICY_DRY_RUN | MT_POLICY_SEE_POSE)) == 0, nm + ".flags: unknown MT_POLICY_* flag");
  const bool auto_reset = (p->flags & MT_POLICY_AUTO_RESET) != 0, dry = (p->flags & MT_POLICY_DRY_RUN) != 0;
  MT_REQUIRE(h, !(auto_reset && dry), nm + ".flags: MT_POLICY_DRY_RUN | MT_POLICY_AUTO_RESET: the re-arm writes the return ring");
  MT_REQUIRE(h, p->n_steps >= 0 && p->n_steps <= 65535, nm + ".n_steps must be 0..65535");
  const int L = p->n_layers;
  MT_REQUIRE(h, L >= 1 && L <= MT_POLICY_MAX_LAYERS, nm + ".n_layers must be 1.." + std::to_string(MT_POLICY_MAX_LAYERS));
  int widest = 0;
  for (int l = 0; l + 1 < L; ++l) {
    MT_REQUIRE(h, p->width[l] >= 1 && p->width[l] <= MT_POLICY_MAX_WIDTH,
               nm + ".width[" + std::to_string(l) + "] must be 1.." + std::to_string(MT_POLICY_MAX_WIDTH));
    widest = std::max(widest, (int)p->width[l]);
  }
  MT_REQUIRE(h, L == 1 || p->hidden_act == MT_ACT_TANH || p->hidden_act == MT_ACT_RELU, nm + ".hidden_act must be MT_ACT_TANH or MT_ACT_RELU");
  MT_REQUIRE(h, p->out_act == MT_ACT_TANH || p->out_act == MT_ACT_IDENTITY, nm + ".out_act must be MT_ACT_TANH or MT_ACT_IDENTITY");
  MT_REQUIRE(h, first_unusable(&p->lo, 1, kMaxAngleBits) < 0 && first_unusable(&p->hi, 1, kMaxAngleBits) < 0,
             nm + ".lo / hi must be finite and within +-32768 degrees");
  MT_REQUIRE(h, p->lo <= p->hi, nm + ".lo must be <= hi");
  MT_REQUIRE(h, first_unusable(&p->out_scale, 1, kMaxFiniteBits) < 0, nm + ".out_scale must be finite");
// ... 618 lines not shown
  MT_REQUIRE(h, s->reward_log != nullptr && s->done_log != nullptr && s->out != nullptr, "mt_reward_to_go.reward_log / done_log / out is NULL");
  MT_REQUIRE(h, s->log_ld >= h->n, "mt_reward_to_go.log_ld is smaller than n_envs");
  MT_REQUIRE(h, s->out_ld >= h->n, "mt_reward_to_go.out_ld is smaller than n_envs");
  const size_t log_bytes = (size_t)(((int64_t)s->n_steps - 1) * s->log_ld + h->n);
  const size_t out_bytes = (size_t)(((int64_t)s->n_steps - 1) * s->out_ld + h->n) * 4;
  MT_REQUIRE(h, !bytes_overlap(s->out, out_bytes, s->reward_log, log_bytes) && !bytes_overlap(s->out, out_bytes, s->done_log, log_bytes),
             "mt_reward_to_go.out overlaps reward_log / done_log");
  MT_ENTER(h);
  RewardToGoArgs r{};
  r.reward = s->reward_log;
  r.done = s->done_log;
  r.log_ld = s->log_ld;
  r.out = s->out;
  r.out_ld = s->out_ld;
  r.n = h->n;
  r.T = s->n_steps;
  r.gamma = s->gamma;
  r.baseline = s->baseline;
  r.mask_after_done = (s->flags & MT_RTG_MASK_AFTER_DONE) ? 1u : 0u;
  hipLaunchKernelGGL(reward_to_go_kernel, grid_for(h->n), dim3(kBlock), 0, h->stream, r);
  return check_launch(h, "reward_to_go_kernel");
}

int mt_shoot(mt_handle h, const struct mt_shoot* s) {
  MT_REQUIRE(nullptr, h != nullptr, "handle is NULL");
  MT_REQUIRE(h, s != nullptr, "shoot is NULL");
  MT_REQUIRE(h, s->struct_size == (int32_t)sizeof(struct mt_shoot), "mt_shoot.struct_size does not match this library");
  MT_REQUIRE(h, s->reserved == 0, "mt_shoot.reserved must be 0");
  MT_REQUIRE(h, (s->flags & ~MT_SHOOT_AUTO_RESET) == 0, "mt_shoot.flags: unknown MT_SHOOT_* flag");
  const bool auto_reset = (s->flags & MT_SHOOT_AUTO_RESET) != 0;
  MT_REQUIRE(h, s->n_steps >= 0, "mt_shoot.n_steps must be >= 0");
  MT_REQUIRE(h, s->n_candidates >= 1 && s->n_candidates <= 64, "mt_shoot.n_candidates must be 1..64");
  MT_REQUIRE(h, s->commit_steps >= 0 && s->commit_steps <= s->n_steps, "mt_shoot.commit_steps must be 0..n_steps");
  MT_REQUIRE(h, !(auto_reset && s->commit_steps == 0), "MT_SHOOT_AUTO_RESET with mt_shoot.commit_steps == 0: an evaluation re-arms nothing");
  if (!fusable(h)) return fail_unfusable(h, "mt_shoot");
  if (!h->is_reset) return fail(h, MT_ERR_STATE, "mt_shoot before mt_reset / mt_reset_random");
  if (s->n_steps == 0) return MT_OK;
  const int H = s->commit_steps;
  MT_REQUIRE(h, s->actions != nullptr, "mt_shoot.actions is NULL");
  MT_REQUIRE(h, s->ld >= h->n, "mt_shoot.ld is smaller than n_envs");
  MT_REQUIRE(h, s->cand_stride >= (int64_t)s->n_steps * h->D * s->ld, "mt_shoot.cand_stride is smaller than n_steps * dof * ld");
  MT_REQUIRE(h, !s->returns_out || s->ret_ld >= h->n, "mt_shoot.ret_ld is smaller than n_envs");
  MT_REQUIRE(h, !(H > 0 && s->best_out == nullptr), "mt_shoot.best_out is NULL with commit_steps > 0");
  MT_REQUIRE(h, !(H > 0 && (s->reward_log || s->done_log)) || s->log_ld >= h->n, "mt_shoot.log_ld is smaller than n_envs");
  MT_ENTER(h);
  ShootArgs e{};
  e.plans = s->actions;
  e.ld = s->ld;
  e.cand_stride = s->cand_stride;
  e.returns_out = s->returns_out;
  e.ret_ld = s->ret_ld;
  e.best_out = s->best_out;
  e.best_return_out = s->best_return_out;
  e.T = s->n_steps;
  e.C = s->n_candidates;
  launch_shoot(h, h->args, e);
  int rc = check_launch(h, "shoot_kernel");
  if (rc || H == 0) return rc;
  TapeArgs r = tape_args(s, s->actions, s->ld, H);
  r.best = s->best_out;
  r.cand_stride = s->cand_stride;
  return commit_tape(h, r, s->seed, auto_reset, true);
}

int mt_sample_plans(mt_handle h, const struct mt_cem* s, void* plans_out, int64_t ld, int64_t cand_stride) {
  MT_REQUIRE(nullptr, h != nullptr, "handle is NULL");
  MT_REQUIRE(h, s != nullptr, "mt_sample_plans: cem is NULL");
  CemArgs e{};
  int rc = stream_args(h, s, "mt_sample_plans: ", kCemNames, e);
  if (rc) return rc;
  if (s->n_steps == 0) return MT_OK;
  rc = stream_rows(h, s, "mt_sample_plans: ", kCemNames);
  if (rc) return rc;
  MT_REQUIRE(h, plans_out != nullptr, "mt_sample_plans: plans_out is NULL");
  MT_REQUIRE(h, ld >= h->n, "mt_sample_plans: ld is smaller than n_envs");
  MT_REQUIRE(h, cand_stride >= (int64_t)s->n_steps * h->D * ld, "mt_sample_plans: cand_stride is smaller than n_steps * dof * ld");
  MT_ENTER(h);
  MT_DISPATCH_D(h->D, launch_sample_plans_d, h, e, static_cast<float*>(plans_out), ld, cand_stride);
  return check_launch(h, "sample_plans_kernel");
}

int mt_cem(mt_handle h, const struct mt_cem* s) {
  MT_REQUIRE(nullptr, h != nullptr, "handle is NULL");
  MT_REQUIRE(h, s != nullptr, "cem is NULL");
  MT_REQUIRE(h, s->struct_size == (int32_t)sizeof(struct mt_cem), "mt_cem.struct_size does not match this library");
  MT_REQUIRE(h, s->reserved == 0, "mt_cem.reserved must be 0");
  CemArgs e{};
  int rc = stream_args(h, s, "mt_cem: ", kCemNames, e);
  if (rc) return rc;
  const bool auto_reset = (s->flags & MT_CEM_AUTO_RESET) != 0;
  const int T = s->n_steps, H = s->commit_steps;
  MT_REQUIRE(h, s->n_elites >= 1 && s->n_elites <= s->n_candidates, "mt_cem.n_elites must be 1..n_candidates");
  MT_REQUIRE(h, H >= 0 && H <= T, "mt_cem.commit_steps must be 0..n_steps");
  MT_REQUIRE(h, !(auto_reset && H == 0), "MT_CEM_AUTO_RESET with mt_cem.commit_steps == 0: an evaluation re-arms nothing");
  MT_REQUIRE(h, first_unusable(&s->sigma_min, 1, kMaxFiniteBits) < 0 && s->sigma_min >= 0.f, "mt_cem.sigma_min must be finite and >= 0");
  if (!fusable(h)) return fail_unfusable(h, "mt_cem");
  if (!h->is_reset) return fail(h, MT_ERR_STATE, "mt_cem before mt_reset / mt_reset_random");
  if (T == 0) return MT_OK;
  rc = stream_rows(h, s, "", kCemNames);
  if (rc) return rc;
  MT_REQUIRE(h, (s->mean_out == nullptr) == (s->sigma_out == nullptr), "mt_cem.mean_out and sigma_out: both or neither");
  rc = refit_args(h, s, kCemNames, e);
  if (rc) return rc;
  MT_ENTER(h);
  e.elite_mask = reinterpret_cast<unsigned long long*>(s->elite_mask_out);
  e.E = s->n_elites;
  e.inv_e = 1.0f / (float)s->n_elites;
  launch_cem(h, h->args, e);
  rc = check_launch(h, "cem_kernel");
  if (rc || H == 0) return rc;
  TapeArgs r = tape_args(s, s->chosen_out, s->chosen_ld, H);
  r.nt_loads = h->tape_nt_loads ? 1u : 0u;
  return commit_tape(h, r, s->seed, auto_reset, false);
}

int mt_mppi(mt_handle h, const struct mt_mppi* s) {
  MT_REQUIRE(nullptr, h != nullptr, "handle is NULL");
  MT_REQUIRE(h, s != nullptr, "mppi is NULL");
  MT_REQUIRE(h, s->struct_size == (int32_t)sizeof(struct mt_mppi), "mt_mppi.struct_size does not match this library");
  MT_REQUIRE(h, s->reserved == 0, "mt_mppi.reserved must be 0");
  MppiArgs e{};
  int rc = stream_args(h, s, "", kMppiNames, e);
  if (rc) return rc;
  const bool auto_reset = (s->flags & MT_MPPI_AUTO_RESET) != 0;
  const int T = s->n_steps, H = s->commit_steps;
  MT_REQUIRE(h, H >= 0 && H <= T, "mt_mppi.commit_steps must be 0..n_steps");
  MT_REQUIRE(h, !(auto_reset && H == 0), "MT_MPPI_AUTO_RESET with mt_mppi.commit_steps == 0: an evaluation re-arms nothing");
  MT_REQUIRE(h, first_unusable(&s->sigma_min, 1, kMaxFiniteBits) < 0 && s->sigma_min >= 0.f, "mt_mppi.sigma_min must be finite and >= 0");
  MT_REQUIRE(h, first_unusable(&s->decay, 1, 0x3F800000u) < 0 && s->decay >= 0.f, "mt_mppi.decay must be finite and within 0..1");
  if (!fusable(h)) return fail_unfusable(h, "mt_mppi");
  if (!h->is_reset) return fail(h, MT_ERR_STATE, "mt_mppi before mt_reset / mt_reset_random");
  if (T == 0) return MT_OK;
  rc = stream_rows(h, s, "", kMppiNames);
  if (rc) return rc;
  MT_REQUIRE(h, !(s->sigma_out && !s->mean_out), "mt_mppi.sigma_out without mean_out");
  rc = refit_args(h, s, kMppiNames, e);
  if (rc) return rc;
  MT_ENTER(h);
  e.weights_out = s->weights_out;
  e.w_ld = s->w_ld;
  e.weight_sum_out = s->weight_sum_out;
  e.decay = s->decay;
  launch_mppi(h, h->args, e);
  rc = check_launch(h, "mppi_kernel");
  if (rc || H == 0) return rc;
  TapeArgs r = tape_args(s, s->chosen_out, s->chosen_ld, H);
  r.nt_loads = h->tape_nt_loads ? 1u : 0u;
  return commit_tape(h, r, s->seed, auto_reset, false);
}

int mt_observe(mt_handle h) {
  MT_REQUIRE(nullptr, h != nullptr, "handle is NULL");
  if (!h->is_reset) return fail(h, MT_ERR_STATE, "mt_observe before reset");
  MT_ENTER(h);
  MT_DISPATCH_D(h->D, launch_observe_d, h);
  return check_launch(h, "observe_kernel");
}

int mt_check_done(mt_handle h) {
  MT_REQUIRE(nullptr, h != nullptr, "handle is NULL");
  if (!h->is_reset) return fail(h, MT_ERR_STATE, "mt_check_done before reset");
  MT_ENTER(h);
  MT_DISPATCH_D(h->D, launch_check_done_d, h);
  return check_launch(h, "check_done_kernel");
}

static int64_t env_major_bytes(mt_handle h, int field) {
  const int64_t n = h->n;
  switch (field) {
    case MT_F_ACTIONS:
    case MT_F_GOALS: return n * h->D * 4;
    case MT_F_POINTS:
    case MT_F_OBS: return n * 3 * h->K * 4;
    case MT_F_ALIVE: return n * h->K;
    case MT_F_REWARD:
    case MT_F_TOTAL_REWARD:
    case MT_F_EPISODES:
    case MT_F_LAST_RETURN: return n * 4;
    case MT_F_DONE: return n;
    case MT_F_DONE_BITS: return (n + 63) / 64 * 8;
    case MT_F_EE: return n * 3 * 4;
    case MT_F_JOINTS: return n * h->D * 3 * 4;
    case MT_F_RETURN_RING: return h->args.ring ? n * (int64_t)h->args.ring_slots * 4 : -1;
    case MT_F_TRACE: return h->trace ? n * (int64_t)h->cfg.substeps * 3 * 4 : -1;
    case MT_F_ZMIN: return h->args.zmin ? n * 4 : -1;
    default: return -1;
  }
}

int mt_get(mt_handle h, int field, void* dst, int64_t dst_bytes, int is_device) {
  MT_REQUIRE(nullptr, h != nullptr, "handle is NULL");
  MT_REQUIRE(h, dst != nullptr, "dst is NULL");
  const int64_t need = env_major_bytes(h, field);
  MT_REQUIRE(h, need > 0, "unknown field (or a field this handle was created without)");
  MT_REQUIRE(h, dst_bytes == need, "dst_bytes does not match the field's env-major size");
  MT_ENTER(h);
  const dim3 g = grid_for(h->n), b(kBlock);
  void* out = dst;
  if (!is_device) {
    int rc = ensure_staging(h, (size_t)need);
    if (rc) return rc;
    out = h->staging;
  }
  const StepArgs& a = h->args;
  bool direct = false;
  const void* direct_src = nullptr;
  switch (field) {
    case MT_F_ACTIONS: hipLaunchKernelGGL((soa_to_env_major<float>), g, b, 0, h->stream, a.actions, h->ld, h->D, h->n, (float*)out); break;
    case MT_F_GOALS: hipLaunchKernelGGL((soa_to_env_major<float>), g, b, 0, h->stream, a.goals, h->ld, h->D, h->n, (float*)out); break;
    case MT_F_POINTS: hipLaunchKernelGGL((soa_to_env_major<float>), g, b, 0, h->stream, a.points, h->ld, 3 * h->K, h->n, (float*)out); break;
    case MT_F_OBS: hipLaunchKernelGGL((soa_to_env_major<float>), g, b, 0, h->stream, a.obs, h->ld, 3 * h->K, h->n, (float*)out); break;
    case MT_F_EE: hipLaunchKernelGGL((soa_to_env_major<float>), g, b, 0, h->stream, a.ee, h->ld, 3, h->n, (float*)out); break;
    case MT_F_RETURN_RING: hipLaunchKernelGGL((soa_to_env_major<float>), g, b, 0, h->stream, a.ring, h->ld, (int)a.ring_slots, h->n, (float*)out); break;
    case MT_F_TRACE: hipLaunchKernelGGL((soa_to_env_major<float>), g, b, 0, h->stream, h->trace, h->ld, 3 * h->cfg.substeps, h->n, (float*)out); break;
    case MT_F_ALIVE: hipLaunchKernelGGL(alive_unpack, g, b, 0, h->stream, a.alive, h->K, h->n, (uint8_t*)out); break;
    case MT_F_JOINTS: MT_DISPATCH_D(h->D, launch_joints_d, h, (float*)out); break;
    case MT_F_REWARD: direct = true; direct_src = a.reward; break;
    case MT_F_TOTAL_REWARD: direct = true; direct_src = a.total_reward; break;
    case MT_F_EPISODES: direct = true; direct_src = a.episodes; break;
    case MT_F_LAST_RETURN: direct = true; direct_src = a.last_return; break;
    case MT_F_DONE: direct = true; direct_src = a.done; break;
    case MT_F_DONE_BITS: direct = true; direct_src = a.done_bits; break;
    case MT_F_ZMIN: direct = true; direct_src = a.zmin; break;
    default: return fail(h, MT_ERR_INVALID_ARG, "unknown field");
  }
  if (direct) {
    MT_HIP(h, hipMemcpyAsync(dst, direct_src, (size_t)need, is_device ? hipMemcpyDeviceToDevice : hipMemcpyDeviceToHost,
                             h->stream));
  } else {
    int rc = check_launch(h, "mt_get transpose");
    if (rc) return rc;
    if (!is_device) MT_HIP(h, hipMemcpyAsync(dst, h->staging, (size_t)need, hipMemcpyDeviceToHost, h->stream));
  }
  if (!is_device) MT_HIP(h, hipStreamSynchronize(h->stream));
  return MT_OK;
}

int mt_set(mt_handle h, int field, const void* src, int64_t src_bytes) {
  MT_REQUIRE(nullptr, h != nullptr, "handle is NULL");
  MT_REQUIRE(h, src != nullptr, "src is NULL");
  MT_REQUIRE(h, field == MT_F_GOALS || field == MT_F_POINTS || field == MT_F_ALIVE || field == MT_F_TOTAL_REWARD ||
                    field == MT_F_DONE || field == MT_F_EPISODES || field == MT_F_LAST_RETURN || field == MT_F_RETURN_RING,
             "field is not settable");
  const int64_t need = env_major_bytes(h, field);
  MT_REQUIRE(h, need > 0, "the handle was created without this field");
  MT_REQUIRE(h, src_bytes == need, "src_bytes does not match the field's env-major size");
  if (field == MT_F_GOALS || field == MT_F_POINTS || field == MT_F_TOTAL_REWARD || field == MT_F_LAST_RETURN ||
      field == MT_F_RETURN_RING) {
    const int64_t bad = first_unusable((const float*)src, need / 4, field == MT_F_GOALS ? kMaxAngleBits : kMaxFiniteBits);
    if (bad >= 0)
      return fail(h, MT_ERR_INVALID_ARG, "mt_set: element " + std::to_string(bad) + " is NaN, infinite or (joint angles) beyond "
                                         "+-32768 degrees");
  }
  MT_ENTER(h);
  const dim3 g = grid_for(h->n), b(kBlock);
  const StepArgs& a = h->args;
  void* row = field == MT_F_TOTAL_REWARD ? (void*)a.total_reward : field == MT_F_DONE ? (void*)a.done :
              field == MT_F_EPISODES ? (void*)a.episodes : field == MT_F_LAST_RETURN ? (void*)a.last_return : nullptr;
  if (field == MT_F_LAST_RETURN || field == MT_F_RETURN_RING) {
    int rcg = order_behind_inplace_gather(h, h->stream);
    if (rcg) return rcg;
  }
  if (row) {
    MT_HIP(h, hipMemcpyAsync(row, src, (size_t)need, hipMemcpyHostToDevice, h->stream));
    if (field == MT_F_DONE) {
      hipLaunchKernelGGL(done_bits_rebuild_kernel, g, b, 0, h->stream, a.done, h->n, a.done_bits);
      int rc = check_launch(h, "done_bits_rebuild_kernel");
      if (rc) return rc;
    }
  } else {
    int rc = ensure_staging(h, (size_t)need);
    if (rc) return rc;
    MT_HIP(h, hipMemcpyAsync(h->staging, src, (size_t)need, hipMemcpyHostToDevice, h->stream));
    if (field == MT_F_GOALS) {
      hipLaunchKernelGGL((env_major_to_soa<float>), g, b, 0, h->stream, (const float*)h->staging, h->D, h->n, a.goals, h->ld);
      h->args.flags &= ~kFlagWholeGoals;
    } else if (field == MT_F_POINTS) {
      hipLaunchKernelGGL((env_major_to_soa<float>), g, b, 0, h->stream, (const float*)h->staging, 3 * h->K, h->n, a.points, h->ld);
      h->codes_valid = false;
    }
    else if (field == MT_F_RETURN_RING)
      hipLaunchKernelGGL((env_major_to_soa<float>), g, b, 0, h->stream, (const float*)h->staging, (int)a.ring_slots, h->n, a.ring, h->ld);
    else
      hipLaunchKernelGGL(alive_pack, g, b, 0, h->stream, (const uint8_t*)h->staging, h->K, h->n, a.alive);
    rc = check_launch(h, "mt_set");
    if (rc) return rc;
  }
  MT_HIP(h, hipStreamSynchronize(h->stream));
  return MT_OK;
}

int mt_set_episode_base(mt_handle h, uint32_t episode0) {
  MT_REQUIRE(nullptr, h != nullptr, "handle is NULL");
  h->args.episode0 = episode0;
  return MT_OK;
}

int mt_device_ptr(mt_handle h, int field, void** ptr, int64_t* rows, int64_t* ld, int* dtype) {
  MT_REQUIRE(nullptr, h != nullptr, "handle is NULL");
  MT_REQUIRE(h, ptr != nullptr, "ptr is NULL");
  FieldInfo fi{};
  int rc = field_info(h, field, &fi);
  if (rc) return rc;
  if (h->reset_pending) {
    MT_ON_DEVICE(h, h->cfg.device);
    rc = flush_pending_reset(h);
    if (rc) return rc;
  }
  h->snap_valid = false;
  if (field == MT_F_GOALS) {
    h->goals_exposed = true;
    h->args.flags &= ~kFlagWholeGoals;
  }
  if (field == MT_F_POINTS) {
    h->points_exposed = true;
    h->codes_valid = false;
  }
  *ptr = fi.ptr;
  if (rows) *rows = fi.rows;
  if (ld) *ld = (field == MT_F_DONE_BITS) ? h->ld / 64 : h->ld;
  if (dtype) *dtype = fi.dtype;
  return MT_OK;
}

int mt_timer_start(mt_handle h) {
  MT_REQUIRE(nullptr, h != nullptr, "handle is NULL");
  MT_ENTER_TIMER(h);
  MT_HIP(h, hipEventRecord(h->ev0, h->stream));
  return MT_OK;
}

int mt_timer_stop(mt_handle h, float* elapsed_ms) {
  MT_REQUIRE(nullptr, h != nullptr, "handle is NULL");
  MT_REQUIRE(h, elapsed_ms != nullptr, "elapsed_ms is NULL");
  MT_ENTER_TIMER(h);
  MT_HIP(h, hipEventRecord(h->ev1, h->stream));
  MT_HIP(h, hipEventSynchronize(h->ev1));
  MT_HIP(h, hipEventElapsedTime(elapsed_ms, h->ev0, h->ev1));
  return MT_OK;
}

int mt_timer_stop_async(mt_handle h) {
  MT_REQUIRE(nullptr, h != nullptr, "handle is NULL");
  MT_ON_DEVICE(h, h->cfg.device);
  MT_HIP(h, hipEventRecord(h->ev1, h->stream));
  h->timer_ends = 1;
  if (h->forked)
    for (int c = 1; c < h->chains; ++c) {
      if (!h->chain_streams[c] || (int64_t)c * chain_span(h, h->chains) >= h->n) continue;
      if (!h->ev1c[c]) MT_HIP(h, hipEventCreateWithFlags(&h->ev1c[c], event_flags(true)));
      MT_HIP(h, hipEventRecord(h->ev1c[c], h->chain_streams[c]));
      h->timer_ends = c + 1;
    }
  h->timer_with_gather = h->gather_pending;
  return MT_OK;
}

int mt_timer_read(mt_handle h, float* elapsed_ms) {
  MT_REQUIRE(nullptr, h != nullptr, "handle is NULL");
  MT_REQUIRE(h, elapsed_ms != nullptr, "elapsed_ms is NULL");
  if (h->timer_ends < 1) return fail(h, MT_ERR_STATE, "mt_timer_read without mt_timer_stop_async");
  MT_ON_DEVICE(h, h->cfg.device);
  float best = 0.f, v = 0.f;
  MT_HIP(h, hipEventSynchronize(h->ev1));
  MT_HIP(h, hipEventElapsedTime(&best, h->ev0, h->ev1));
  for (int c = 1; c < h->timer_ends; ++c) {
    if (!h->ev1c[c]) continue;
    MT_HIP(h, hipEventSynchronize(h->ev1c[c]));
    MT_HIP(h, hipEventElapsedTime(&v, h->ev0, h->ev1c[c]));
    best = v > best ? v : best;
  }
  if (h->timer_with_gather && h->ev_g1) {
    MT_HIP(h, hipEventSynchronize(h->ev_g1));
    if (hipEventElapsedTime(&v, h->ev0, h->ev_g1) == hipSuccess)
      best = v > best ? v : best;
    else
      (void)hipGetLastError();
  }
  *elapsed_ms = best;
  h->timer_ends = 0;
  return MT_OK;
}

static int lap_reserve(mt_handle h, size_t count) {
  while (h->lap_events.size() < h->lap_events_used + count) {
    hipEvent_t e = nullptr;
    MT_HIP(h, hipEventCreateWithFlags(&e, event_flags(true)));
    h->lap_events.push_back(e);
  }
  return MT_OK;
}

static int lap_event(mt_handle h, hipStream_t stream, uint32_t* index) {
  int rcr = lap_reserve(h, 1);
  if (rcr) return rcr;
  MT_HIP(h, hipEventRecord(h->lap_events[h->lap_events_used], stream));
  *index = (uint32_t)h->lap_events_used++;
  return MT_OK;
}

int mt_timer_lap_begin(mt_handle h) {
  MT_REQUIRE(nullptr, h != nullptr, "handle is NULL");
  if (h->lap_open) return fail(h, MT_ERR_STATE, "mt_timer_lap_begin: a lap is already open");
  const bool per_chain = h->forked && h->lazy_chains && h->stream == h->own_stream;
  if (per_chain) {
    MT_ON_DEVICE(h, h->cfg.device);
    int rcf = flush_pending_reset(h);
    if (rcf) return rcf;
  } else {
    MT_ENTER(h);
  }
  mt_engine::LapRec rec{0, 1, 0, 0};
  int rc = lap_reserve(h, 2 * (size_t)mt_engine::kMaxChains);
  if (rc) return rc;
  rc = lap_event(h, h->stream, &rec.begin);
  if (rc) return rc;
  if (per_chain && h->forked)
    for (int c = 1; c < h->chains; ++c) {
      if (!h->chain_streams[c] || (int64_t)c * chain_span(h, h->chains) >= h->n) continue;
      uint32_t idx;
      rc = lap_event(h, h->chain_streams[c], &idx);
      if (rc) return rc;
      ++rec.n_begin;
    }
  h->lap_recs.push_back(rec);
  h->lap_open = true;
  return MT_OK;
}

int mt_timer_lap_end(mt_handle h) {
  MT_REQUIRE(nullptr, h != nullptr, "handle is NULL");
  if (!h->lap_open) return fail(h, MT_ERR_STATE, "mt_timer_lap_end without mt_timer_lap_begin");
  MT_ON_DEVICE(h, h->cfg.device);
  mt_engine::LapRec& rec = h->lap_recs.back();
  int rc = lap_event(h, h->stream, &rec.end0);
  if (rc) return rc;
  rec.n_end = 1;
  if (h->forked)
    for (int c = 1; c < h->chains; ++c) {
      if (!h->chain_streams[c] || (int64_t)c * chain_span(h, h->chains) >= h->n) continue;
      uint32_t idx;
      rc = lap_event(h, h->chain_streams[c], &idx);
      if (rc) return rc;
      ++rec.n_end;
    }
  h->lap_open = false;
  return MT_OK;
}

static int lap_ms(mt_handle h, const mt_engine::LapRec& rec, float* ms) {
  float best = 0.f;
  for (uint32_t k = 0; k < rec.n_end; ++k) {
    MT_HIP(h, hipEventSynchronize(h->lap_events[rec.end0 + k]));
    for (uint32_t b = 0; b < rec.n_begin; ++b) {
      float v = 0.f;
      MT_HIP(h, hipEventElapsedTime(&v, h->lap_events[rec.begin + b], h->lap_events[rec.end0 + k]));
      best = v > best ? v : best;
    }
  }
  *ms = best;
  return MT_OK;
}

int mt_timer_lap_times(mt_handle h, float* ms, int capacity, int* n_laps) {
  MT_REQUIRE(nullptr, h != nullptr, "handle is NULL");
  MT_REQUIRE(h, n_laps != nullptr && (ms != nullptr || capacity == 0), "NULL argument");
  if (h->lap_open) return fail(h, MT_ERR_STATE, "mt_timer_lap_times: a lap is still open");
  const size_t laps = h->lap_recs.size();
  *n_laps = (int)laps;
  if ((size_t)capacity < laps) return fail(h, MT_ERR_INVALID_ARG, "mt_timer_lap_times: capacity is smaller than the number of laps");
  MT_ON_DEVICE(h, h->cfg.device);
  for (size_t i = 0; i < laps; ++i) {
    int rc = lap_ms(h, h->lap_recs[i], &ms[i]);
    if (rc) return rc;
  }
  h->lap_recs.clear();
  h->lap_events_used = 0;
  return MT_OK;
}

int mt_timer_laps_total(mt_handle h, float* total_ms, int* n_laps) {
  MT_REQUIRE(nullptr, h != nullptr, "handle is NULL");
  MT_REQUIRE(h, total_ms != nullptr, "total_ms is NULL");
  if (h->lap_open) return fail(h, MT_ERR_STATE, "mt_timer_laps_total: a lap is still open");
  MT_ON_DEVICE(h, h->cfg.device);
  double sum = 0.0;
  for (const auto& rec : h->lap_recs) {
    float v = 0.f;
    int rc = lap_ms(h, rec, &v);
    if (rc) return rc;
    sum += v;
  }
  *total_ms = (float)sum;
  if (n_laps) *n_laps = (int)h->lap_recs.size();
  h->lap_recs.clear();
  h->lap_events_used = 0;
  return MT_OK;
}

namespace {
struct Scratch {
  void* p = nullptr;
  size_t bytes = 0;
};
std::mutex g_scratch_mu;
Scratch g_scratch[64];

int scratch_reserve(int device, size_t bytes, void** out) {
  if (device < 0 || device >= 64) return fail(nullptr, MT_ERR_INVALID_ARG, "device ordinal out of range");
  Scratch& sc = g_scratch[device];
  if (sc.bytes < bytes) {
    if (sc.p) (void)hipFree(sc.p);
    sc.p = nullptr;
    sc.bytes = 0;
    const size_t want = align_up(bytes, (size_t)1 << 16);
    if (hipMalloc(&sc.p, want) != hipSuccess) {
      (void)hipGetLastError();
      sc.p = nullptr;
      return fail(nullptr, MT_ERR_ALLOC, "hipMalloc of the helper scratch failed");
    }
    sc.bytes = want;
  }
  *out = sc.p;
  return MT_OK;
}
}

int mt_fk_batch(int device, const float* dh_table, int dof, int mode, const float* angles, int angles_in_radians,
                int64_t n, float* out_mat16) {
  MT_REQUIRE(nullptr, dh_table && angles && out_mat16, "NULL argument");
  MT_REQUIRE(nullptr, dof >= 1 && dof <= MT_MAX_DOF && mode >= 0 && mode <= dof, "dof/mode out of range");
  MT_REQUIRE(nullptr, n >= 1, "n must be >= 1");
  MT_REQUIRE(nullptr, first_unusable(dh_table, (int64_t)dof * 4, kMaxFiniteBits) < 0 && first_unusable(angles, n * dof, kMaxFiniteBits) < 0,
             "mt_fk_batch: NaN or infinity in dh_table / angles");
  MT_ON_DEVICE(nullptr, device);
  std::lock_guard<std::mutex> lock(g_scratch_mu);
  const size_t in_b = align_up((size_t)n * dof * 4, 256);
  void* base = nullptr;
  int rc = scratch_reserve(device, in_b + (size_t)n * 64, &base);
  if (rc) return rc;
  float* d_in = (float*)base;
  float* d_out = (float*)((char*)base + in_b);
  FkArgs a{d_in, d_out, n, dof, mode, angles_in_radians, make_dh(dh_table, dof)};
  hipError_t e = hipMemcpy(d_in, angles, (size_t)n * dof * 4, hipMemcpyHostToDevice);
  if (e == hipSuccess) {
    hipLaunchKernelGGL(fk_kernel, grid_for(n), dim3(kBlock), 0, 0, a);
    e = hipGetLastError();
  }
  if (e == hipSuccess) e = hipMemcpy(out_mat16, d_out, (size_t)n * 64, hipMemcpyDeviceToHost);
  if (e != hipSuccess) rc = fail(nullptr, MT_ERR_HIP, std::string("mt_fk_batch: ") + hipGetErrorString(e));
  return rc;
}

int mt_route_trace(int device, const float* dh_table, int dof, int substeps, const float* prev, const float* action,
                   int64_t n, float* out) {
  MT_REQUIRE(nullptr, dh_table && prev && action && out, "NULL argument");
  MT_REQUIRE(nullptr, dof >= 2 && dof <= MT_MAX_DOF && substeps >= 2, "dof/substeps out of range");
  MT_REQUIRE(nullptr, n >= 1 && n * substeps < ((int64_t)1 << 31), "n out of range");
  MT_REQUIRE(nullptr, first_unusable(dh_table, (int64_t)dof * 4, kMaxFiniteBits) < 0 && first_unusable(prev, n * dof, kMaxFiniteBits) < 0 &&
                          first_unusable(action, n * dof, kMaxFiniteBits) < 0,
             "mt_route_trace: NaN or infinity in dh_table / prev / action");
  MT_ON_DEVICE(nullptr, device);
  const size_t in_b = align_up((size_t)n * dof * 4, 256), out_b = (size_t)n * substeps * dof * 3 * 4;
// ... 98 lines not shown
```

manytor_amd/csrc/engine_internal.h:

```cpp
#pragma once
#include <hip/hip_runtime.h>

#include <cstdlib>
#include <string>
#include <vector>

#include "step_args.h"

struct mt_comm;

struct mt_engine {
  static constexpr int kMaxChains = 4;
  mt_config cfg{};
  int64_t n = 0, ld = 0;
  int D = 0, K = 0;
  hipStream_t own_stream = nullptr;
  hipStream_t stream = nullptr;
  hipEvent_t ev0 = nullptr, ev1 = nullptr;
  hipEvent_t ev1c[kMaxChains] = {nullptr, nullptr, nullptr, nullptr};
  int timer_ends = 0;
  bool timer_with_gather = false;
  struct LapRec {
    uint32_t begin, n_begin, end0, n_end;
  };
  std::vector<hipEvent_t> lap_events;
  size_t lap_events_used = 0;
  std::vector<LapRec> lap_recs;
  bool lap_open = false;
  void* arena = nullptr;
  size_t arena_bytes = 0;
  void* staging = nullptr;
  size_t staging_bytes = 0;
  void* pinned = nullptr;
  size_t pinned_bytes = 0;
  mt::StepArgs args{};
  float* trace = nullptr;
  unsigned long long* spare_bits = nullptr;
  bool is_reset = false;
  int trig = 0;
  bool lds_table = false;
  bool custom_frames = false;
  struct Schedule {
    int step_lanes = 1;
    bool prefetch = false;
    int rollout_lanes = 1;
  };
  enum Scope { kBatch = 0, kChain = 1, kOneEnv = 2 };
  Schedule sched[2];
  int blocks_per_cu_override = -1;
  int64_t flat_from = 393216;
  bool goals_exposed = false;
  bool codes_valid = false;
  bool points_exposed = false;
  bool trig_steps = false;
  int static_kind = 0;
  mt_comm* comm = nullptr;
  hipStream_t side_stream = nullptr;
  hipEvent_t ev_snap = nullptr, ev_g0 = nullptr, ev_g1 = nullptr;
  float* snap = nullptr;
  hipEvent_t ev_gdone[2] = {nullptr, nullptr};
  bool snap_free_known[2] = {true, true};
  int snap_next = 0;
  bool gather_throttle = true;
  float* snap_row(int p) const { return snap + (size_t)p * (size_t)n; }
  void* reduce_scratch = nullptr;
  size_t reduce_scratch_bytes = 0;
  bool reset_split = false;
  struct RolloutGraph {
    int T;
    int chains;
    mt::StepArgs args;
    hipGraphExec_t exec[kMaxChains];
  };
  std::vector<RolloutGraph> graphs;
  std::vector<int> graph_seen;
  uint32_t* graph_step0 = nullptr;
  int graph_mode = -1;
  int64_t graph_max = 131072;
  int chains = 1;
  bool chains_forced = false;
  int multi_k = 1;
  bool rollout_early = true;
  bool defer_reset_chained = false;
  bool defer_reset = true;
  bool reset_pending = false;
  uint64_t pend_seed = 0;
  uint32_t pend_episode = 0;
  bool snap_in_rollout = true;
  bool snap_valid = false;
  bool tape_prefetch = false;
  bool tape_nt_loads = false;
  bool ground_compact = true;
  std::string overrides;
  std::string describe;
  hipStream_t chain_streams[kMaxChains] = {nullptr, nullptr, nullptr, nullptr};
  hipEvent_t ev_fork = nullptr, ev_join[kMaxChains] = {nullptr, nullptr, nullptr, nullptr};
  bool forked = false;
  bool lazy_chains = true;
  bool gather_pending = false;
  bool gather_inplace = false;
  float last_gather_ms = 0.f;
  int cu_count = 0;
  std::string err;
  std::string kernel_name;
};

namespace mt {

inline unsigned event_flags(bool timing) {
  static const bool fenced = [] {
    const char* e = std::getenv("MT_EVENT_FENCE");
    return e && *e && std::atoi(e) != 0;
  }();
  return (timing ? 0u : (unsigned)hipEventDisableTiming) | (fenced ? 0u : (unsigned)hipEventDisableSystemFence);
}

int fail(mt_handle h, int code, const std::string& msg);

class DeviceGuard {
 public:
  explicit DeviceGuard(int device) {
    if (hipGetDevice(&prev_) != hipSuccess) prev_ = -1;
    err_ = (prev_ == device) ? hipSuccess : hipSetDevice(device);
    changed_ = (err_ == hipSuccess && prev_ != device);
  }
  ~DeviceGuard() {
    if (changed_ && prev_ >= 0) (void)hipSetDevice(prev_);
  }
  hipError_t error() const { return err_; }

 private:
  int prev_ = -1;
  hipError_t err_ = hipSuccess;
  bool changed_ = false;
};

inline dim3 grid_for(int64_t n) { return dim3((unsigned)((n + kBlock - 1) / kBlock)); }

inline bool snapshot_trusted(mt_engine* h) {
  if (h->stream != h->own_stream) return false;
  hipStreamCaptureStatus st = hipStreamCaptureStatusNone;
  if (hipStreamIsCapturing(h->stream, &st) != hipSuccess) {
    (void)hipGetLastError();
    return false;
  }
  return st == hipStreamCaptureStatusNone;
}

int join_chains(mt_handle h);
int flush_pending_reset(mt_handle h);

}

#define MT_HIP(h, call)                                                                            \
  do {                                                                                             \
    hipError_t e__ = (call);                                                                       \
    if (e__ != hipSuccess)                                                                         \
      return mt::fail(h, MT_ERR_HIP, std::string(#call) + ": " + hipGetErrorString(e__));          \
  } while (0)

#define MT_REQUIRE(h, cond, msg)                              \
  do {                                                        \
    if (!(cond)) return mt::fail(h, MT_ERR_INVALID_ARG, msg); \
  } while (0)

#define MT_ON_DEVICE(h, device)                                                                          \
  mt::DeviceGuard mt_guard__(device);                                                                    \
  if (mt_guard__.error() != hipSuccess)                                                                  \
  return mt::fail(h, MT_ERR_HIP, std::string("hipSetDevice: ") + hipGetErrorString(mt_guard__.error()))

#define MT_ENTER(h)                              \
  MT_ON_DEVICE(h, (h)->cfg.device);              \
  do {                                           \
    (h)->snap_valid = false;                     \
    if ((h)->forked) {                           \
      int rcj__ = mt::join_chains(h);            \
      if (rcj__ != MT_OK) return rcj__;          \
    }                                            \
    if ((h)->reset_pending) {                    \
      int rcf__ = mt::flush_pending_reset(h);    \
      if (rcf__ != MT_OK) return rcf__;          \
    }                                            \
  } while (0)

#define MT_ENTER_TIMER(h)                        \
  MT_ON_DEVICE(h, (h)->cfg.device);              \
  do {                                           \
    if ((h)->forked) {                           \
      int rcj__ = mt::join_chains(h);            \
      if (rcj__ != MT_OK) return rcj__;          \
    }                                            \
  } while (0)

void mt_comm_release(mt_handle h);
void mt_gather_release(mt_handle h);
```

manytor_amd/csrc/kernels.h:

```cpp
#pragma once
#include <hip/hip_runtime.h>
#include <stdint.h>

#include <type_traits>

#include "mt_math.h"
#include "philox.h"
#include "step_args.h"

namespace mt {

#ifndef MT_NT_STORES
#define MT_NT_STORES 1
#endif
template <typename T>
using global_ptr = __attribute__((address_space(1))) T*;

__device__ __forceinline__ global_ptr<char> uniform_row(const void* row) {
  const uint64_t v = reinterpret_cast<uint64_t>(row);
  const uint32_t lo = __builtin_amdgcn_readfirstlane((uint32_t)v);
  const uint32_t hi = __builtin_amdgcn_readfirstlane((uint32_t)(v >> 32));
  return (global_ptr<char>)(((uint64_t)hi << 32) | lo);
}
#ifndef MT_PLAIN_LANE_OFFSET
// ... 661 lines not shown
  float zres[2 * kCap];
  float field[kFields][kCap];
};

template <class Tbl>
__device__ __forceinline__ float half_route_zmin(const Tbl& t, float (&s)[Tbl::D], float (&c)[Tbl::D], const float (&sd)[Tbl::D],
                                                 const float (&cd)[Tbl::D], int n_half, int mine) {
  constexpr int D = Tbl::D;
  constexpr int JN = ZJoints<Tbl>::value;
  float zm = 3.0e38f, zo, ze;
#pragma unroll 2
  for (int it = 1; it <= n_half; ++it) {
    rotate_pose<D, JN, +1>(s, c, sd, cd);
    chain_z<Tbl>(s, c, t, zo, ze);
    if (it <= mine) zm = fminf(zm, fminf(zo, ze));
  }
  return zm;
}

struct NoGroundQueue {
  uint32_t count;
};
__device__ __forceinline__ void ground_queue_reset(uint32_t* count) {
  if (threadIdx.x == 0) *count = 0u;
}

template <class Tbl, bool TABLE>
__device__ __forceinline__ float route_kinematics_block(const Tbl& t, int S, float inv_sm1, const float (&g)[Tbl::D],
                                                        const float (&act)[Tbl::D], float (&el)[3], float (&e)[3],
                                                        const SinCos* trig, bool prev_whole, bool live, GroundQueue<Tbl>& q) {
  constexpr int D = Tbl::D;
  constexpr int JN = ZJoints<Tbl>::value;
  constexpr int kCap = GroundQueue<Tbl>::kCap;
  const int nf = (S - 1) / 2;
  const int nb = S - 2 - nf;
  float zmin;
  bool undecided = false;
  float sF[D], cF[D], sA[D], cA[D], sd[D], cd[D];
  if (__builtin_expect(__any(live && wide_route<Tbl, TABLE>(g, act, prev_whole)), 0)) {
    zmin = route_kinematics_wide<Tbl, false>(t, S, g, act, el, e, nullptr);
  } else {
    float st[D];
#pragma unroll
    for (int j = 0; j < D; ++j) st[j] = (act[j] - g[j]) * inv_sm1;
    float p[D][3], zo, ze;
    action_sincos<Tbl, TABLE>(t, act, sA, cA, trig);
    chain_all<Tbl>(sA, cA, t, p);
    pick_frames<Tbl>(t, p, el, e);
    zmin = fminf(el[2], e[2]);
#pragma unroll
    for (int j = 0; j < D; ++j) {
      sF[j] = 0.f;
      cF[j] = 1.f;
    }
    prev_pose_sincos<Tbl, TABLE>(t, g, sF, cF, trig, prev_whole);
    chain_z<Tbl>(sF, cF, t, zo, ze);
    zmin = fminf(zmin, fminf(zo, ze));
    sincos_increment<D, JN>(st, sd, cd);
    sA[0] = 0.f;
    cA[0] = 1.f;
    undecided = live && !(zmin < 0.f);
  }

  const unsigned long long um = __ballot(undecided);
  uint32_t slot = kCap;
  if (um != 0ull) {
    uint32_t base = 0u;
    if ((threadIdx.x & 63u) == 0u) base = atomicAdd(&q.count, (uint32_t)__popcll(um));
    base = (uint32_t)__builtin_amdgcn_readfirstlane((int)base);
    slot = base + __builtin_amdgcn_mbcnt_hi((uint32_t)(um >> 32), __builtin_amdgcn_mbcnt_lo((uint32_t)um, 0u));
  }
  const bool queued = undecided && slot < (uint32_t)kCap;
  if (queued) {
#pragma unroll
    for (int j = 1; j < JN; ++j) {
      float(*f)[kCap] = q.field + 6 * (j - 1);
      f[0][slot] = sF[j];
      f[1][slot] = cF[j];
      f[2][slot] = sA[j];
      f[3][slot] = cA[j];
      f[4][slot] = sd[j];
      f[5][slot] = cd[j];
    }
  }
  if (undecided && !queued) {
    zmin = fminf(zmin, half_route_zmin<Tbl>(t, sF, cF, sd, cd, nf, nf));
#pragma unroll
    for (int j = 1; j < JN; ++j) sd[j] = -sd[j];
    zmin = fminf(zmin, half_route_zmin<Tbl>(t, sA, cA, sd, cd, nf, nb));
  }
  __syncthreads();

  const uint32_t routes = q.count < (uint32_t)kCap ? q.count : (uint32_t)kCap;
  const uint32_t w = (threadIdx.x + 64u * (blockIdx.x & 3u)) & (uint32_t)(kBlock - 1);
  if (w < 2u * routes) {
    const uint32_t r = w >> 1;
    const bool backward = (w & 1u) != 0u;
    float sW[D], cW[D], sdW[D], cdW[D];
#pragma unroll
    for (int j = 0; j < D; ++j) {
      sW[j] = 0.f;
      cW[j] = 1.f;
      sdW[j] = 0.f;
      cdW[j] = 1.f;
    }
#pragma unroll
    for (int j = 1; j < JN; ++j) {
      const float(*f)[kCap] = q.field + 6 * (j - 1);
      sW[j] = backward ? f[2][r] : f[0][r];
      cW[j] = backward ? f[3][r] : f[1][r];
      const float sdj = f[4][r];
      sdW[j] = backward ? -sdj : sdj;
      cdW[j] = f[5][r];
    }
    q.zres[w] = half_route_zmin<Tbl>(t, sW, cW, sdW, cdW, nf, backward ? nb : nf);
  }
  __syncthreads();
  if (queued) zmin = fminf(zmin, fminf(q.zres[2u * slot], q.zres[2u * slot + 1u]));
  return zmin;
}

__device__ __forceinline__ void record_finished(const StepArgs& a, uint32_t i, uint32_t episode, float ret) {
  LaneOffset<true> o4{i * 4u};
  str(a.last_return, o4, ret);
  if (a.ring_slots)
    a.ring[(int64_t)((episode - a.episode0) % a.ring_slots) * a.ld + i] = ret;
}

#ifdef MT_STAMPS
#define MT_STAMP(a, i, slot)                                                                 \
  do {                                                                                       \
    __builtin_amdgcn_sched_barrier(0);                                                       \
    unsigned long long t__;                                                                  \
    asm volatile("s_memtime %0\n\ts_waitcnt lgkmcnt(0)" : "=s"(t__)::"memory");              \
    __builtin_amdgcn_sched_barrier(0);                                                       \
    if ((a).stamps && (threadIdx.x & 63) == 0) (a).stamps[(size_t)((i) >> 6) * 8 + (slot)] = t__; \
  } while (0)
#else
#define MT_STAMP(a, i, slot) \
  do {                       \
  } while (0)
#endif

__device__ __forceinline__ bool unusable_angle(float v) { return (__float_as_uint(v) & 0x7FFFFFFFu) > 0x47000000u; }

template <class Tbl, int TRIG>
constexpr int step_min_waves() { return (TRIG == 0 && Tbl::D >= 6 && Tbl::D <= 7) ? 8 : 1; }

constexpr int kPrefetch = 8;

__device__ __forceinline__ void draw_targets_wave(uint64_t seed, uint64_t env0, uint32_t episode, bool need, int K, float radius,
                                                  float* col0, uint8_t* slots);

template <class Tbl, bool SAMPLE, int TRIG, bool LDS, int PF = 0, bool TT = false, bool FLAT = false, bool FRESH = false,
          bool CODES = false, bool GC = false>
__global__ __launch_bounds__(kBlock, (PF ? 1 : step_min_waves<Tbl, TRIG>())) void step_kernel(const StepArgs a) {
  constexpr int D = Tbl::D;
  static_assert(!GC || (TRIG == 0 && !LDS && !FRESH), "the block-cooperative ground test serves the recurrence");
  static_assert(!TT || (SAMPLE && TRIG == 0 && !LDS && ActionTrigTable<Tbl>::value), "the table serves sampled actions of a static table");
  static_assert(!FRESH || TT, "the reset prologue exists for the sampled-action kernels of the static tables");
  static_assert(!CODES || (PF && TT && !FRESH), "codes are read by the prefetch kernels of the static tables");
  extern __shared__ float fresh_stage[];
  __shared__ uint8_t fresh_slots[FRESH ? kBlock / 64 : 1][64];
  __shared__ DhConst sh;
  __shared__ __attribute__((aligned(16))) SinCos trig_lds[TT ? kTrigEntries : 1];
  __shared__ std::conditional_t<GC, GroundQueue<Tbl>, NoGroundQueue> ground_q;
  float4 trig_v;
  if (TT) trig_v = trig_table_load(a.trig_table);
  if constexpr (GC) {
    ground_queue_reset(&ground_q.count);
    if (!TT) __syncthreads();
  }
  if (LDS) {
    const float* src = reinterpret_cast<const float*>(&a.dh);
    float* dst = reinterpret_cast<float*>(&sh);
    if (threadIdx.x < sizeof(DhConst) / sizeof(float)) dst[threadIdx.x] = src[threadIdx.x];
    __syncthreads();
  }
  const Tbl t = TableMaker<Tbl>::make(LDS ? sh : a.dh);

  const uint32_t i = blockIdx.x * kBlock + threadIdx.x;
  LaneOffset<!FLAT> o4{i * 4u}, o1{i};
  const bool live = i < a.n;
  if (!TT && !GC && !live) return;
  const int64_t ld = a.ld;
  const uint32_t step_no = SAMPLE ? step_index(a) : 0u;

  constexpr bool kLean = D >= 6;
  MT_STAMP(a, i, 0);
  float g[D], act[D];
#pragma unroll
  for (int j = 0; j < D; ++j) g[j] = FRESH ? 0.f : ldr(a.goals + j * ld, o4);
  float tx[PF ? PF : 1][3];
  uint32_t tc[CODES ? PF : 1][2];
  if constexpr (FRESH) {
    const bool mine = i < a.n;
    const uint32_t lane = threadIdx.x & 63u;
    if (mine) {
      str(a.last_return, o4, ldr(a.total_reward, o4));
      str(a.episodes, o4, a.reset_episode);
    }
    draw_targets_wave(((uint64_t)a.reset_seed_hi << 32) | a.reset_seed_lo, (uint64_t)(a.env_base + (i - lane)), a.reset_episode, mine,
                      a.K, a.radius, fresh_stage + (threadIdx.x - lane), fresh_slots[threadIdx.x >> 6]);
    if (mine) {
      const float* col = fresh_stage + threadIdx.x;
#pragma unroll
      for (int k = 0; k < (PF ? PF : 0); ++k)
        if (k < a.K) {
          decode_target(staged_code(col + 2 * k * kBlock, kBlock), a.radius, tx[k][0], tx[k][1], tx[k][2]);
#pragma unroll
          for (int q = 0; q < 3; ++q) str(a.points + (int64_t)(3 * k + q) * ld, o4, tx[k][q]);
        }
      for (int k = PF; k < a.K; ++k) {
        float x, y, z;
        decode_target(staged_code(col + 2 * k * kBlock, kBlock), a.radius, x, y, z);
        const int64_t r = 3 * k;
        str(a.points + r * ld, o4, x);
        str(a.points + (r + 1) * ld, o4, y);
        str(a.points + (r + 2) * ld, o4, z);
      }
    }
  } else if (PF) {
#pragma unroll
    for (int k = 0; k < PF; ++k)
      if (k < a.K) {
        if constexpr (CODES) {
          const uint32_t* crow = a.codes + (int64_t)(2 * k) * ld;
          tc[k][0] = ldr(crow, o4);
          tc[k][1] = ldr(crow + ld, o4);
        } else {
          const float* row = a.points + (int64_t)(3 * k) * ld;
#pragma unroll
          for (int q = 0; q < 3; ++q) tx[k][q] = ldr(row + q * ld, o4);
        }
      }
  }
  uint32_t am = 0;
  float total_in = 0.f;
  if (FRESH) {
    am = all_alive_mask(a.K);
  } else if (!kLean || PF) {
    am = ldr(a.alive, o4);
    total_in = ldr(a.total_reward, o4);
  }
  if (SAMPLE) {
    draw_action<D>(((uint64_t)a.seed_hi << 32) | a.seed_lo, (uint64_t)(a.env_base + i), step_no, act);
  } else {
    bool bad = false;
#pragma unroll
    for (int j = 0; j < D; ++j) {
      act[j] = ldr(a.actions + j * ld, o4);
      bad |= unusable_angle(act[j]);
    }
    if (bad) {
#pragma unroll
      for (int j = 0; j < D; ++j) act[j] = g[j];
      if (!GC || live) atomicAdd(a.bad_actions, 1u);
    }
  }
  if constexpr (GC) {
#pragma unroll
    for (int j = 0; j < D; ++j) {
      g[j] = live ? g[j] : 0.f;
      if (!SAMPLE) act[j] = live ? act[j] : 0.f;
    }
  }
  MT_STAMP(a, i, 1);
  if (TT) {
    trig_table_commit(trig_lds, trig_v);
    if (!GC && !live) return;
  }
  if (kLean && (!GC || live)) {
#pragma unroll
    for (int j = 0; j < D; ++j) str(a.goals + j * ld, o4, act[j]);
  }

  float el[3], e[3];
  float zmin;
  if constexpr (GC) {
    zmin = route_kinematics_block<Tbl, TT>(t, a.S, a.inv_sm1, g, act, el, e, trig_lds, (a.flags & kFlagWholeGoals) != 0, live,
                                           ground_q);
    if (!live) return;
  } else {
    zmin = route_kinematics<Tbl, TRIG, false, TT>(t, a.S, a.inv_sm1, g, act, el, e, nullptr, false, trig_lds,
                                                  (a.flags & kFlagWholeGoals) != 0);
  }
  const bool ground = zmin < 0.f;
  if (a.zmin) str_stream(a.zmin, o4, zmin);
  if (kLean && !PF && !FRESH) {
    am = ldr(a.alive, o4);
    total_in = ldr(a.total_reward, o4);
  }
  MT_STAMP(a, i, 2);

  uint32_t nam = am;
  if (PF) {
#pragma unroll
    for (int k = 0; k < PF; ++k)
      if (k < a.K) {
        if constexpr (CODES) decode_target(TargetCode{tc[k][0], tc[k][1]}, a.radius, tx[k][0], tx[k][1], tx[k][2]);
        step_target<false, CODES>(a, ld, o4, k, am, nam, el, e, tx[k][0], tx[k][1], tx[k][2]);
      }
  }
  for (int k = PF; k < a.K; ++k) {
    if (TRIG == 5) {
      float dist, r, th;
      const float x = (float)(i & 63) + (float)k, y = 3.0f + (float)k, z = 5.0f + g[0];
      observe_target(el, x, y, z, dist, r, th);
      if (within_box(e, x, y, z, a.tol)) nam &= ~(1u << k);
      if (dist + r + th == -12345.0f) (a.obs + (int64_t)(3 * k) * ld)[i] = dist;
      continue;
    }
    if constexpr (CODES) {
      const uint32_t* crow = a.codes + (int64_t)(2 * k) * ld;
      float x, y, z;
      decode_target(TargetCode{ldr(crow, o4), ldr(crow + ld, o4)}, a.radius, x, y, z);
      step_target<false, true>(a, ld, o4, k, am, nam, el, e, x, y, z);
      continue;
    }
    const float* row = a.points + (int64_t)(3 * k) * ld;
    {
      const float x = ldr(row, o4), y = ldr(row + ld, o4), z = ldr(row + 2 * ld, o4);
      step_target<TRIG == 4>(a, ld, o4, k, am, nam, el, e, x, y, z);
    }
  }

  MT_STAMP(a, i, 3);
  const int32_t rew = ground ? -1 : ((nam != am) ? 1 : 0);
  bool done = (nam == 0u);
  if (a.flags & MT_FLAG_TERMINATE_ON_GROUND) done |= ground;

  if (!kLean) {
#pragma unroll
    for (int j = 0; j < D; ++j) str(a.goals + j * ld, o4, act[j]);
  }
#pragma unroll
  for (int q = 0; q < 3; ++q) str_stream(a.ee + q * ld, o4, e[q]);
  str(a.alive, o4, nam);
  str_stream(a.reward, o4, rew);
  str(a.total_reward, o4, total_in + (float)rew);
  if (a.snap) str(a.snap, o4, total_in + (float)rew);
  str_stream(a.done, o1, (uint8_t)(done ? 1 : 0));
  const unsigned long long bits = __ballot(done);
  if ((threadIdx.x & 63) == 0) a.done_bits[i >> 6] = bits;
  MT_STAMP(a, i, 4);
#ifdef MT_STAMPS
  asm volatile("s_waitcnt vmcnt(0)" ::: "memory");
  MT_STAMP(a, i, 5);
#endif
}

template <class Tbl, int L, bool CACHED, bool TABLE>
__device__ __forceinline__ float route_kinematics_split_narrow(const Tbl& t, int S, float inv_sm1, const float (&g)[Tbl::D],
                                                               const float (&act)[Tbl::D], bool backward, float (&el)[3],
                                                               float (&e)[3], PoseCache<Tbl::D>* cache, bool cache_valid,
                                                               const SinCos* trig, bool prev_whole) {
  constexpr int D = Tbl::D;
  constexpr int JN = ZJoints<Tbl>::value;
  constexpr int EPW = 64 / L;
  const bool use_cache = CACHED && __all(cache_valid);
  float st[D];
#pragma unroll
  for (int j = 0; j < D; ++j) st[j] = (act[j] - g[j]) * inv_sm1;
  float sA[D], cA[D], p3[D][3];
  action_sincos<Tbl, TABLE>(t, act, sA, cA, trig);
  chain_all<Tbl>(sA, cA, t, p3);
  pick_frames<Tbl>(t, p3, el, e);
  float sF[D], cF[D];
#pragma unroll
  for (int j = 0; j < D; ++j) {
    sF[j] = 0.f;
    cF[j] = 1.f;
  }
  float zo, ze, z0;
  if (use_cache) {
#pragma unroll
    for (int j = 1; j < JN; ++j) {
      sF[j] = cache->s[j];
      cF[j] = cache->c[j];
    }
    z0 = cache->zmin;
  } else {
    prev_pose_sincos<Tbl, TABLE>(t, g, sF, cF, trig, prev_whole);
    chain_z<Tbl>(sF, cF, t, zo, ze);
    z0 = fminf(zo, ze);
  }
  if (CACHED) {
#pragma unroll
    for (int j = 1; j < JN; ++j) {
      cache->s[j] = sA[j];
      cache->c[j] = cA[j];
    }
    cache->zmin = fminf(el[2], e[2]);
  }
  float zmin = backward ? fminf(el[2], e[2]) : z0;
  float sd[D], cd[D];
  sincos_increment<D, JN>(st, sd, cd);
  float sW[D], cW[D];
  sW[0] = 0.f;
  cW[0] = 1.f;
#pragma unroll
  for (int j = 1; j < D; ++j) {
    sW[j] = backward ? sA[j] : sF[j];
    cW[j] = backward ? cA[j] : cF[j];
    sd[j] = backward ? -sd[j] : sd[j];
  }
  const int nf = (S - 1) / 2;
  const int nb = S - 2 - nf;
  const int mine = backward ? nb : nf;
#pragma unroll 2
  for (int it = 1; it <= nf; ++it) {
    rotate_pose<D, JN, +1>(sW, cW, sd, cd);
    chain_z<Tbl>(sW, cW, t, zo, ze);
    if (it <= mine) zmin = fminf(zmin, fminf(zo, ze));
  }
#pragma unroll
  for (int sh = EPW; sh < 64; sh <<= 1) zmin = fminf(zmin, __shfl_xor(zmin, sh));
  return zmin;
}

template <class Tbl, int L, bool CACHED, bool TABLE = false>
__device__ __forceinline__ float route_kinematics_split(const Tbl& t, int S, float inv_sm1, const float (&g)[Tbl::D],
                                                        const float (&act)[Tbl::D], bool backward, float (&el)[3],
                                                        float (&e)[3], PoseCache<Tbl::D>* cache = nullptr,
                                                        bool cache_valid = false, const SinCos* trig = nullptr,
                                                        bool prev_whole = false) {
  if (__builtin_expect(__any(wide_route<Tbl, TABLE>(g, act, prev_whole)), 0))
    return route_kinematics_wide<Tbl, CACHED>(t, S, g, act, el, e, cache);
  return route_kinematics_split_narrow<Tbl, L, CACHED, TABLE>(t, S, inv_sm1, g, act, backward, el, e, cache, cache_valid, trig,
                                                              prev_whole);
}

template <class Tbl, bool SAMPLE, int L, bool TT = false>
__global__ __launch_bounds__(kBlock) void step_split_kernel(const StepArgs a) {
  static_assert(L == 2 || L == 4, "an env is spread over 2 or 4 lanes");
  static_assert(!TT || (SAMPLE && ActionTrigTable<Tbl>::value), "the table serves sampled actions of a static table");
  constexpr int D = Tbl::D;
  constexpr int EPW = 64 / L;
// ... 2525 lines not shown
```

Measured before the change: 32.47 billion.

## Re-derive previous arm pose from the RNG instead of loading goals from memory

Adds host-side tracking of what each chain's goals buffer holds: zeros after a reset, or the random action drawn at the previous step with a known seed. When the state is known, the sampled-action kernel sets the previous pose to zero or recomputes it with draw_action for step-1, so it no longer reads D floats per env from HBM. Tracking is cleared on any other API entry, on graph capture, on rollouts and on exposed or foreign goals. The change is on by default for the ref4 table and chain 0 only. It trades extra RNG arithmetic for less memory traffic and adds a lot of state-invalidation bookkeeping that must stay correct.

```diff
diff --git a/manytor_amd/csrc/engine.hip b/manytor_amd/csrc/engine.hip
--- a/manytor_amd/csrc/engine.hip
+++ b/manytor_amd/csrc/engine.hip
@@ -114,6 +114,10 @@
   int multi_step_k = 5;
   bool fold_reset_into_chains = false;
   int max_recurrence_rotations = 12;
+  bool rederive_goals_ref4 = true;
+  bool rederive_goals_dh7 = false;
+  int rederive_goals_chains = 1;
+  int64_t rederive_goals_max_envs = 3145728;
   int64_t ld_pad_above = 16384;
   int ld_pad_floats = 256;
 };
@@ -258,6 +262,16 @@
   if (env_int("MT_GROUND_COMPACT", &v)) {
     h->ground_compact = v != 0;
     seen("MT_GROUND_COMPACT");
+  }
+
+  h->goals_rederive = h->static_kind == 1 ? P.rederive_goals_ref4 : (h->static_kind == 2 ? P.rederive_goals_dh7 : false);
+  h->goals_rederive_chains = P.rederive_goals_chains;
+  h->goals_rederive_max_envs = P.rederive_goals_max_envs;
+  if (env_int("MT_GOALS_REDERIVE", &v)) {
+    h->goals_rederive = v != 0 && h->static_kind != 0;
+    h->goals_rederive_chains = mt_engine::kMaxChains;
+    h->goals_rederive_max_envs = INT64_MAX;
+    seen("MT_GOALS_REDERIVE");
   }
 
   if (h->custom_frames) h->lds_table = false;
@@ -299,10 +313,11 @@
   bool fresh = false;
   bool codes = false;
   bool gc = false;
+  int prev = kPrevLoad;
 };
 constexpr unsigned variant_key(const StepVariant& v) {
   return (unsigned)v.trig | (unsigned)v.lds << 3 | (unsigned)v.lanes << 4 | (unsigned)(v.pf != 0) << 7 | (unsigned)v.tt << 8 |
-         (unsigned)v.flat << 9 | (unsigned)v.fresh << 10 | (unsigned)v.codes << 11 | (unsigned)v.gc << 12;
+         (unsigned)v.flat << 9 | (unsigned)v.fresh << 10 | (unsigned)v.codes << 11 | (unsigned)v.gc << 12 | (unsigned)v.prev << 13;
 }
 
 #pragma clang diagnostic push
@@ -327,6 +342,12 @@
     {.gc = true}, {.pf = kPrefetch, .gc = true}, {.pf = kPrefetch, .flat = true, .gc = true},
     {.pf = 0, .tt = true, .gc = true}, {.pf = kPrefetch, .tt = true, .gc = true}, {.pf = kPrefetch, .tt = true, .flat = true, .gc = true},
     {.pf = kPrefetch, .tt = true, .codes = true, .gc = true}, {.pf = kPrefetch, .tt = true, .flat = true, .codes = true, .gc = true},
+    {.pf = kPrefetch, .tt = true, .codes = true, .prev = kPrevZero}, {.pf = kPrefetch, .tt = true, .flat = true, .codes = true, .prev = kPrevZero},
+    {.pf = kPrefetch, .tt = true, .codes = true, .prev = kPrevDraw}, {.pf = kPrefetch, .tt = true, .flat = true, .codes = true, .prev = kPrevDraw},
+    {.pf = kPrefetch, .tt = true, .codes = true, .gc = true, .prev = kPrevZero},
+    {.pf = kPrefetch, .tt = true, .flat = true, .codes = true, .gc = true, .prev = kPrevZero},
+    {.pf = kPrefetch, .tt = true, .codes = true, .gc = true, .prev = kPrevDraw},
+    {.pf = kPrefetch, .tt = true, .flat = true, .codes = true, .gc = true, .prev = kPrevDraw},
 };
 #pragma clang diagnostic pop
 
@@ -356,7 +377,8 @@
   return bytes;
 }
 
-StepPlan plan_step(const mt_engine* h, mt_engine::Scope scope, int64_t n, bool sample, bool codes, bool fresh = false) {
+StepPlan plan_step(const mt_engine* h, mt_engine::Scope scope, int64_t n, bool sample, bool codes, bool fresh = false,
+                   int prev = kPrevLoad) {
   const mt_engine::Schedule& s = h->sched[scope == mt_engine::kChain ? mt_engine::kChain : mt_engine::kBatch];
   const bool whole_rows = scope != mt_engine::kOneEnv;
   StepPlan p;
@@ -400,6 +422,7 @@
   v.pf = s.prefetch ? kPrefetch : 0;
   v.flat = v.pf && n >= h->flat_from;
   v.codes = v.pf && v.tt && codes;
+  v.prev = v.codes ? prev : kPrevLoad;
   v.gc = ground_compacts(h, whole_rows);
   if (v.pf && v.tt) {
     p.blocks_per_cu = step_blocks_per_cu(h, n);
@@ -414,8 +437,8 @@
   if constexpr (V.lanes > 1)
     hipLaunchKernelGGL((step_split_kernel<Tbl, SAMPLE, V.lanes, V.tt>), p.grid, dim3(kBlock), p.lds_bytes, stream, args);
   else
-    hipLaunchKernelGGL((step_kernel<Tbl, SAMPLE, V.trig, V.lds, V.pf, V.tt, V.flat, V.fresh, V.codes, V.gc>), p.grid, dim3(kBlock),
-                       p.lds_bytes, stream, args);
+    hipLaunchKernelGGL((step_kernel<Tbl, SAMPLE, V.trig, V.lds, V.pf, V.tt, V.flat, V.fresh, V.codes, V.gc, V.prev>), p.grid,
+                       dim3(kBlock), p.lds_bytes, stream, args);
 }
 template <class Tbl, const auto& ROWS, size_t I>
 bool launch_row(const StepPlan& p, hipStream_t stream, const StepArgs& args) {
@@ -471,20 +494,54 @@
     hipLaunchKernelGGL((trace_kernel<D, false>), grid_for(args.n), dim3(kBlock), 0, h->stream, args, trace);
 }
 
-void launch_step(mt_handle h, mt_engine::Scope scope, const StepArgs& args, float* trace, bool sample) {
+static bool goals_tracked(const mt_engine* h, const StepArgs& args) {
+  return !h->goals_exposed && !h->goals_foreign && !args.major_base;
+}
+
+static int goals_prev(const mt_engine* h, mt_engine::Scope scope, const StepArgs& args, bool traced, bool sample, int chain) {
+  if (!sample || traced || scope == mt_engine::kOneEnv || !goals_tracked(h, args)) return -1;
+  mt_engine::GoalsRow r = h->goals_row[chain >= 0 ? chain : 0];
+  if (chain < 0)
+    for (int c = 1; c < h->chains; ++c)
+      if (h->goals_row[c].kind != r.kind || h->goals_row[c].seed != r.seed || h->goals_row[c].step != r.step) r = mt_engine::GoalsRow{};
+  if (!h->goals_rederive || chain >= h->goals_rederive_chains || args.n > h->goals_rederive_max_envs) return kPrevLoad;
+  if (r.kind == mt_engine::GoalsRow::kZero) return kPrevZero;
+  const uint64_t seed = ((uint64_t)args.seed_hi << 32) | args.seed_lo;
+  if (r.kind == mt_engine::GoalsRow::kDraw && r.seed == seed && r.step + 1u == args.major && args.major != 0u) return kPrevDraw;
+  return kPrevLoad;
+}
+
+void launch_step(mt_handle h, mt_engine::Scope scope, const StepArgs& args, float* trace, bool sample, int chain = -1) {
   if (trace) MT_DISPATCH_D(h->D, launch_trace_d, h, args, trace, sample);
-  const StepPlan p = plan_step(h, scope, args.n, sample, h->codes_valid);
+  const int prev = goals_prev(h, scope, args, trace != nullptr, sample, chain);
+  const StepPlan p = plan_step(h, scope, args.n, sample, h->codes_valid, false, prev < 0 ? (int)kPrevLoad : prev);
   launch_plan(p, h->stream, args);
   h->codes_valid = p.v.codes;
+  if (p.v.prev != kPrevLoad) ++h->goals_rederived;
+  const mt_engine::GoalsRow row =
+      (prev >= 0 && sample && p.v.lanes == 1)
+          ? mt_engine::GoalsRow{mt_engine::GoalsRow::kDraw, args.major, ((uint64_t)args.seed_hi << 32) | args.seed_lo}
+          : mt_engine::GoalsRow{};
+  if (chain >= 0)
+    h->goals_row[chain] = row;
+  else
+    for (mt_engine::GoalsRow& g : h->goals_row) g = row;
 }
 
 void launch_step(mt_handle h, bool sample) { launch_step(h, mt_engine::kBatch, h->args, h->trace, sample); }
 
-bool launch_step_fresh(mt_handle h, mt_engine::Scope scope, const StepArgs& args) {
+bool launch_step_fresh(mt_handle h, mt_engine::Scope scope, const StepArgs& args, int chain) {
   const StepPlan p = plan_step(h, scope, args.n, true, false, true);
   if (!p.exists) return false;
   launch_plan(p, h->stream, args);
   h->codes_valid = p.v.codes;
+  const mt_engine::GoalsRow row = goals_tracked(h, args)
+                                      ? mt_engine::GoalsRow{mt_engine::GoalsRow::kDraw, args.major, ((uint64_t)args.seed_hi << 32) | args.seed_lo}
+                                      : mt_engine::GoalsRow{};
+  if (chain >= 0)
+    h->goals_row[chain] = row;
+  else
+    for (mt_engine::GoalsRow& g : h->goals_row) g = row;
   return true;
 }
 
@@ -505,7 +562,7 @@
   StepArgs as = args_for_range(h, a0, off, std::min(span, h->n - off));
   for (int s = 0; s < T; ++s) {
     as.major = major0 + (uint32_t)s;
-    launch_step(h, mt_engine::kChain, as, nullptr, sample);
+    launch_step(h, mt_engine::kChain, as, nullptr, sample, c);
   }
 }
 
@@ -514,7 +571,7 @@
   if (off >= h->n) return true;
   StepArgs as = args_for_range(h, a0, off, std::min(span, h->n - off));
   as.major = major;
-  return launch_step_fresh(h, mt_engine::kChain, as);
+  return launch_step_fresh(h, mt_engine::kChain, as, c);
 }
 
 hipStream_t chain_stream(mt_handle h, int c) { return c == 0 ? h->stream : h->chain_streams[c]; }
@@ -640,6 +697,7 @@
 }
 void launch_rollout(mt_handle h, const StepArgs& a, int lanes, const RolloutArgs& r, bool early = false) {
   h->codes_valid = false;
+  h->forget_goals();
   if (h->static_kind == 1) return early ? launch_rollout_t<Ref4Table, kPrefetch>(h, a, lanes, r) : launch_rollout_t<Ref4Table, 0>(h, a, lanes, r);
   if (h->static_kind == 2) return early ? launch_rollout_t<Dh7Table, kPrefetch>(h, a, lanes, r) : launch_rollout_t<Dh7Table, 0>(h, a, lanes, r);
   MT_DISPATCH_D(h->D, launch_rollout_d, h, a, lanes, r);
@@ -1208,6 +1266,10 @@
   const StepPlan sb = batch_plan(h), sc = chain_plan(h);
   const bool multi = h->multi_k > 1 && fusable(h);
   const bool graph = h->graph_mode > 0 || (h->graph_mode < 0 && h->n <= h->graph_max);
+  const bool rederive_on = h->goals_rederive && !h->goals_exposed && !h->goals_foreign && !h->points_exposed && !h->trace;
+  auto rederives = [&](const StepPlan& p) {
+    return rederive_on && p.v.lanes == 1 && p.v.pf != 0 && p.v.tt && (&p == &sb ? h->n : span) <= h->goals_rederive_max_envs;
+  };
   std::string caps = "[";
   for (const BlockCap& c : P.block_caps) caps += std::string(caps.size() > 1 ? "," : "") + "[" + num(c.from) + "," + num(c.below) + "," + num(c.blocks) + "]";
   caps += "]";
@@ -1235,6 +1297,10 @@
       ",\"policy_rollout\":{\"usable\":" + b(fusable(h)) + ",\"lanes_per_env\":1,\"hidden_extents\":[32,64]}" +
       ",\"reset\":{\"lanes_per_env\":" + num(h->reset_split ? 4 : 1) + "}" +
       ",\"ground_compact\":{\"enabled\":" + b(h->ground_compact) + ",\"step\":" + b(sb.v.gc) + ",\"chains\":" + b(sc.v.gc) + "}" +
+      ",\"goals\":{\"rederive\":" + b(!multi && !graph && rederives(h->chains > 1 ? sc : sb)) + ",\"enabled\":" + b(h->goals_rederive) +
+      ",\"step\":" + b(rederives(sb)) + ",\"chains\":" + b(rederives(sc)) +
+      ",\"chains_rederiving\":" + num(rederives(sc) ? std::min(h->chains, h->goals_rederive_chains) : 0) +
+      ",\"launches_rederived\":" + num((long long)h->goals_rederived) + "}" +
       ",\"overrides\":\"" + h->overrides + "\"" +
       ",\"policy\":{\"step_split4_max\":" + num(P.step_split4_max) + ",\"step_split2_max\":" + num(P.step_split2_max) +
       ",\"prefetch_other_max\":" + num(P.prefetch_other_max) + ",\"fused_split4_max\":" + num(P.fused_split4_max) +
@@ -1244,7 +1310,9 @@
       ",\"chain_prefetch_other_max\":" + num(P.chain_prefetch_other_max) + ",\"flat_from\":" + num(P.flat_from) +
       ",\"block_caps\":" + caps + ",\"multi_step_max\":" + num(P.multi_step_max) + ",\"multi_step_k\":" + num(P.multi_step_k) +
       ",\"max_recurrence_rotations\":" + num(P.max_recurrence_rotations) + ",\"ld_pad_above\":" + num(P.ld_pad_above) +
-      ",\"ld_pad_floats\":" + num(P.ld_pad_floats) + "}" +
+      ",\"ld_pad_floats\":" + num(P.ld_pad_floats) + ",\"rederive_goals_ref4\":" + b(P.rederive_goals_ref4) +
+      ",\"rederive_goals_dh7\":" + b(P.rederive_goals_dh7) + ",\"rederive_goals_chains\":" + num(P.rederive_goals_chains) +
+      ",\"rederive_goals_max_envs\":" + num(P.rederive_goals_max_envs) + "}" +
       ",\"arena_bytes\":" + num((long long)h->arena_bytes) + "}";
   return d.c_str();
 }
@@ -1267,7 +1335,7 @@
 
 int mt_sync(mt_handle h) {
   MT_REQUIRE(nullptr, h != nullptr, "handle is NULL");
-  MT_ENTER(h);
+  MT_ENTER_KEEP(h);
   MT_HIP(h, hipStreamSynchronize(h->stream));
   if (h->gather_pending) {
     MT_HIP(h, hipStreamSynchronize(h->side_stream));
@@ -1322,6 +1390,7 @@
   MT_DISPATCH_D(h->D, launch_reset_d, h, h->args, 0);
   int rc = check_launch(h, "reset_kernel");
   if (rc) return rc;
+  h->goals_are(mt_engine::GoalsRow::kZero);
   if (!is_device) MT_HIP(h, hipStreamSynchronize(h->stream));
   h->is_reset = true;
   return MT_OK;
@@ -1340,6 +1409,7 @@
     h->args.episode0 = episode;
     if (!h->goals_exposed) h->args.flags |= kFlagWholeGoals;
   }
+  h->forget_goals();
   if (per_chain) {
     int rc = fork_chains(h, h->chains);
     if (rc) return rc;
@@ -1357,6 +1427,7 @@
     if (rc == MT_OK) rc = check_launch(h, "reset_kernel (per chain)");
     if (rc) return rc;
     h->codes_valid = !h->points_exposed;
+    h->goals_are(mt_engine::GoalsRow::kZero);
     h->is_reset = true;
     return settle_chains(h);
   }
@@ -1365,7 +1436,10 @@
   MT_DISPATCH_D(h->D, launch_reset_d, h, h->args, mode);
   rc = check_launch(h, "reset_kernel");
   if (rc) return rc;
-  if (mode == 1) h->codes_valid = !h->points_exposed;
+  if (mode == 1) {
+    h->codes_valid = !h->points_exposed;
+    h->goals_are(mt_engine::GoalsRow::kZero);
+  }
   h->is_reset = true;
   return MT_OK;
 }
@@ -1386,6 +1460,7 @@
   MT_REQUIRE(nullptr, h != nullptr, "handle is NULL");
   MT_ON_DEVICE(h, h->cfg.device);
   h->snap_valid = false;
+  note_capture(h);
   int rc = flush_pending_reset(h);
   if (rc) return rc;
   if (mode == 1 && h->defer_reset && h->stream == h->own_stream &&
@@ -1395,6 +1470,7 @@
     h->args.major = episode;
     h->args.episode0 = episode;
     if (!h->goals_exposed) h->args.flags |= kFlagWholeGoals;
+    h->forget_goals();
     h->reset_pending = true;
     h->pend_seed = seed;
     h->pend_episode = episode;
@@ -1512,6 +1588,7 @@
   if (chains > 1) {
     MT_ON_DEVICE(h, h->cfg.device);
     h->snap_valid = false;
+    note_capture(h);
     {
       int rcf = flush_pending_reset(h);
       if (rcf) return rcf;
@@ -1582,7 +1659,7 @@
 int mt_step_random(mt_handle h, uint64_t seed, uint32_t step_idx) {
   MT_REQUIRE(nullptr, h != nullptr, "handle is NULL");
   if (!h->is_reset) return fail(h, MT_ERR_STATE, "mt_step_random before mt_reset / mt_reset_random");
-  MT_ENTER(h);
+  MT_ENTER_KEEP(h);
   h->args.seed_lo = (uint32_t)seed;
   h->args.seed_hi = (uint32_t)(seed >> 32);
   h->args.major = step_idx;
@@ -1648,7 +1725,7 @@
 int mt_bad_action_count(mt_handle h, uint64_t* count) {
   MT_REQUIRE(nullptr, h != nullptr, "handle is NULL");
   MT_REQUIRE(h, count != nullptr, "count is NULL");
-  MT_ENTER(h);
+  MT_ENTER_KEEP(h);
   uint32_t c = 0;
   MT_HIP(h, hipMemcpyAsync(&c, h->args.bad_actions, 4, hipMemcpyDeviceToHost, h->stream));
   MT_HIP(h, hipStreamSynchronize(h->stream));
@@ -1742,6 +1819,7 @@
   if (n_steps > 0 && !h->is_reset) return fail(h, MT_ERR_STATE, "mt_rollout before mt_reset / mt_reset_random");
   if (n_steps == 0) return MT_OK;
   MT_ON_DEVICE(h, h->cfg.device);
+  note_capture(h);
   int chains = (n_steps >= 2 || h->reset_pending) ? usable_chains(h) : 1;
   h->snap_valid = false;
   const bool multi = (n_steps >= 2 || h->reset_pending) && rollout_is_multi_step(h);
@@ -1835,6 +1913,7 @@
   if (graph) {
     const mt_engine::RolloutGraph* rg = nullptr;
     h->codes_valid = false;
+    h->forget_goals();
     int rc = rollout_graph(h, n_steps, seed, chains, &rg);
     if (rc) return rc;
     if (chains > 1) {
@@ -2759,7 +2838,7 @@
 int mt_observe(mt_handle h) {
   MT_REQUIRE(nullptr, h != nullptr, "handle is NULL");
   if (!h->is_reset) return fail(h, MT_ERR_STATE, "mt_observe before reset");
-  MT_ENTER(h);
+  MT_ENTER_KEEP(h);
   MT_DISPATCH_D(h->D, launch_observe_d, h);
   return check_launch(h, "observe_kernel");
 }
@@ -2767,7 +2846,7 @@
 int mt_check_done(mt_handle h) {
   MT_REQUIRE(nullptr, h != nullptr, "handle is NULL");
   if (!h->is_reset) return fail(h, MT_ERR_STATE, "mt_check_done before reset");
-  MT_ENTER(h);
+  MT_ENTER_KEEP(h);
   MT_DISPATCH_D(h->D, launch_check_done_d, h);
   return check_launch(h, "check_done_kernel");
 }
@@ -2801,7 +2880,7 @@
   const int64_t need = env_major_bytes(h, field);
   MT_REQUIRE(h, need > 0, "unknown field (or a field this handle was created without)");
   MT_REQUIRE(h, dst_bytes == need, "dst_bytes does not match the field's env-major size");
-  MT_ENTER(h);
+  MT_ENTER_KEEP(h);
   const dim3 g = grid_for(h->n), b(kBlock);
   void* out = dst;
   if (!is_device) {
@@ -3015,7 +3094,7 @@
     int rcf = flush_pending_reset(h);
     if (rcf) return rcf;
   } else {
-    MT_ENTER(h);
+    MT_ENTER_KEEP(h);
   }
   mt_engine::LapRec rec{0, 1, 0, 0};
   int rc = lap_reserve(h, 2 * (size_t)mt_engine::kMaxChains);
diff --git a/manytor_amd/csrc/engine_internal.h b/manytor_amd/csrc/engine_internal.h
--- a/manytor_amd/csrc/engine_internal.h
+++ b/manytor_amd/csrc/engine_internal.h
@@ -52,6 +52,24 @@
   bool goals_exposed = false;
   bool codes_valid = false;
   bool points_exposed = false;
+  struct GoalsRow {
+    enum Kind : uint8_t { kUnknown = 0, kZero = 1, kDraw = 2 };
+    Kind kind = kUnknown;
+    uint32_t step = 0;
+    uint64_t seed = 0;
+  };
+  GoalsRow goals_row[kMaxChains];
+  void forget_goals() {
+    for (GoalsRow& g : goals_row) g = GoalsRow{};
+  }
+  void goals_are(GoalsRow::Kind kind, uint64_t seed = 0, uint32_t step = 0) {
+    for (GoalsRow& g : goals_row) g = GoalsRow{kind, step, seed};
+  }
+  bool goals_rederive = true;
+  int goals_rederive_chains = kMaxChains;
+  int64_t goals_rederive_max_envs = INT64_MAX;
+  bool goals_foreign = false;
+  uint64_t goals_rederived = 0;
   bool trig_steps = false;
   int static_kind = 0;
   mt_comm* comm = nullptr;
@@ -147,6 +165,17 @@
   return st == hipStreamCaptureStatusNone;
 }
 
+inline void note_capture(mt_engine* h) {
+  if (h->goals_foreign || h->stream == h->own_stream) return;
+  hipStreamCaptureStatus st = hipStreamCaptureStatusNone;
+  if (hipStreamIsCapturing(h->stream, &st) != hipSuccess) {
+    (void)hipGetLastError();
+    h->goals_foreign = true;
+  } else if (st != hipStreamCaptureStatusNone) {
+    h->goals_foreign = true;
+  }
+}
+
 int join_chains(mt_handle h);
 int flush_pending_reset(mt_handle h);
 
@@ -169,10 +198,13 @@
   if (mt_guard__.error() != hipSuccess)                                                                  \
   return mt::fail(h, MT_ERR_HIP, std::string("hipSetDevice: ") + hipGetErrorString(mt_guard__.error()))
 
-#define MT_ENTER(h)                              \
+#define MT_ENTER(h) MT_ENTER_IMPL(h, true)
+#define MT_ENTER_KEEP(h) MT_ENTER_IMPL(h, false)
+#define MT_ENTER_IMPL(h, forget)                 \
   MT_ON_DEVICE(h, (h)->cfg.device);              \
   do {                                           \
     (h)->snap_valid = false;                     \
+    mt::note_capture(h);                         \
     if ((h)->forked) {                           \
       int rcj__ = mt::join_chains(h);            \
       if (rcj__ != MT_OK) return rcj__;          \
@@ -181,6 +213,7 @@
       int rcf__ = mt::flush_pending_reset(h);    \
       if (rcf__ != MT_OK) return rcf__;          \
     }                                            \
+    if (forget) (h)->forget_goals();             \
   } while (0)
 
 #define MT_ENTER_TIMER(h)                        \
diff --git a/manytor_amd/csrc/kernels.h b/manytor_amd/csrc/kernels.h
--- a/manytor_amd/csrc/kernels.h
+++ b/manytor_amd/csrc/kernels.h
@@ -837,10 +837,12 @@
 __device__ __forceinline__ void draw_targets_wave(uint64_t seed, uint64_t env0, uint32_t episode, bool need, int K, float radius,
                                                   float* col0, uint8_t* slots);
 
+enum : int { kPrevLoad = 0, kPrevZero = 1, kPrevDraw = 2 };
 template <class Tbl, bool SAMPLE, int TRIG, bool LDS, int PF = 0, bool TT = false, bool FLAT = false, bool FRESH = false,
-          bool CODES = false, bool GC = false>
+          bool CODES = false, bool GC = false, int PREV = kPrevLoad>
 __global__ __launch_bounds__(kBlock, (PF ? 1 : step_min_waves<Tbl, TRIG>())) void step_kernel(const StepArgs a) {
   constexpr int D = Tbl::D;
+  static_assert(PREV == kPrevLoad || CODES, "the previous pose is re-derived by the code-reading kernels (the HBM-bound launches)");
   static_assert(!GC || (TRIG == 0 && !LDS && !FRESH), "the block-cooperative ground test serves the recurrence");
   static_assert(!TT || (SAMPLE && TRIG == 0 && !LDS && ActionTrigTable<Tbl>::value), "the table serves sampled actions of a static table");
   static_assert(!FRESH || TT, "the reset prologue exists for the sampled-action kernels of the static tables");
@@ -874,8 +876,12 @@
   constexpr bool kLean = D >= 6;
   MT_STAMP(a, i, 0);
   float g[D], act[D];
-#pragma unroll
-  for (int j = 0; j < D; ++j) g[j] = FRESH ? 0.f : ldr(a.goals + j * ld, o4);
+  if constexpr (PREV == kPrevDraw) {
+    draw_action<D>(((uint64_t)a.seed_hi << 32) | a.seed_lo, (uint64_t)(a.env_base + i), step_no - 1u, g);
+  } else {
+#pragma unroll
+    for (int j = 0; j < D; ++j) g[j] = (FRESH || PREV == kPrevZero) ? 0.f : ldr(a.goals + j * ld, o4);
+  }
   float tx[PF ? PF : 1][3];
   uint32_t tc[CODES ? PF : 1][2];
   if constexpr (FRESH) {
@@ -962,13 +968,12 @@
 
   float el[3], e[3];
   float zmin;
+  const bool prev_whole = PREV != kPrevLoad || (a.flags & kFlagWholeGoals) != 0;
   if constexpr (GC) {
-    zmin = route_kinematics_block<Tbl, TT>(t, a.S, a.inv_sm1, g, act, el, e, trig_lds, (a.flags & kFlagWholeGoals) != 0, live,
-                                           ground_q);
+    zmin = route_kinematics_block<Tbl, TT>(t, a.S, a.inv_sm1, g, act, el, e, trig_lds, prev_whole, live, ground_q);
     if (!live) return;
   } else {
-    zmin = route_kinematics<Tbl, TRIG, false, TT>(t, a.S, a.inv_sm1, g, act, el, e, nullptr, false, trig_lds,
-                                                  (a.flags & kFlagWholeGoals) != 0);
+    zmin = route_kinematics<Tbl, TRIG, false, TT>(t, a.S, a.inv_sm1, g, act, el, e, nullptr, false, trig_lds, prev_whole);
   }
   const bool ground = zmin < 0.f;
   if (a.zmin) str_stream(a.zmin, o4, zmin);
```

Result: faster. 33.34 billion (median of 6 runs) (+2.7%).
